# NVIDIA-Merlin/NVTabular

Measured on AMD Instinct MI355X. Metric: rows/sec + GB/s (Criteo Categorify+FillMissing+Normalize fit+transform, HBM-resident), higher is better.
Workload: dtype int32 keys -> int64 labels; fp64 moments/normalize; 1 GPU; synthetic Criteo-day0: 26 int32 categorical (Criteo-1TB cardinalities, Zipf) + 13 int32 continuous, nulls as Arrow bitmaps; Categorify + FillMissing + Normalize, fit + transform; rows_per_gpu=45000000, algorithmic_bytes_per_row=624, tie_break=value (count desc, value asc), artifacts=deferred (no parquet I/O inside the timed region)

## Files before the change

### include/nvt_hip.h

```cpp
#ifndef NVT_HIP_H
#define NVT_HIP_H

#include <stdint.h>

#ifdef __cplusplus
extern "C" {
#endif

#define NVT_OK 0
#define NVT_EINVAL (-1)
#define NVT_EHIP (-2)
#define NVT_ENOMEM (-3)
#define NVT_EUNSUPPORTED (-4)

#define NVT_F32 0
#define NVT_F64 1
#define NVT_I32 2
#define NVT_I64 3
#define NVT_U8 4
#define NVT_I8 5
#define NVT_I16 6

#define NVT_EMPTY_I32 INT32_MIN
#define NVT_EMPTY_I64 INT64_MIN
// ... 278 lines not shown
int nvt_keydir_lookup_image(const void *keys, int dtype, const uint8_t *valid, uint64_t n,
                            const uint32_t *dir, uint64_t dir_slots, const int32_t *keys32, uint64_t nkeys,
                            int64_t key_offset, int64_t null_group, const void *image,
                            uint32_t stride_bytes, int ncols, void *const *outs, const uint8_t *const *folds, const uint32_t *offs,
                            const uint32_t *sizes, const uint64_t *miss_bits, uint64_t *unseen,
                            void *stream);
int nvt_image_build(const nvt_image_part *parts, int nparts, uint64_t records, void *image,
                    uint32_t stride_bytes, void *stream);

int nvt_pq_decode_chunk(const uint8_t *chunk, uint64_t chunk_bytes, int type_size, int max_def_level,
                        uint64_t expect_rows, uint8_t *valid_out, uint64_t valid_bit_offset,
                        uint8_t *values_out, uint64_t values_cap_bytes, uint64_t *rows_out,
                        uint64_t *values_count);
int nvt_pq_decode_chunk_codec(const uint8_t *chunk, uint64_t chunk_bytes, int codec, int type_size,
                              int max_def_level, uint64_t expect_rows, uint8_t *valid_out,
                              uint64_t valid_bit_offset, uint8_t *values_out, uint64_t values_cap_bytes,
                              uint8_t *scratch, uint64_t scratch_bytes, uint64_t *rows_out,
                              uint64_t *values_count);
int nvt_pq_decode_list_chunk(const uint8_t *chunk, uint64_t chunk_bytes, int codec, int type_size,
                             int leaf_level, int max_def_level, uint64_t expect_slots, uint64_t expect_rows,
                             uint8_t *rep_out, uint8_t *def_out, uint64_t slot_offset, uint64_t slot_cap,
                             uint8_t *values_out, uint64_t values_cap_bytes, uint8_t *scratch,
                             uint64_t scratch_bytes, uint64_t *counts);
#define NVT_PQ_RUN_REPEAT 0u
#define NVT_PQ_RUN_PACKED 1u
#define NVT_PQ_RUN_SEQUENCE 2u
#define NVT_PQ_RUN_END 3u
#define NVT_PQ_STR_GROW 1
typedef struct nvt_pq_str_stage {
  int64_t *offsets;
  uint8_t *chars;
  uint32_t *runs;
  uint8_t *packed;
  uint64_t entries_cap, chars_cap, runs_cap, packed_cap;
  uint64_t entries, nchars, nruns, npacked, nvalues;
} nvt_pq_str_stage;
int nvt_pq_decode_str_chunk(const uint8_t *chunk, uint64_t chunk_bytes, int codec, int max_def_level,
                            uint64_t expect_rows, uint8_t *valid_out, uint64_t valid_bit_offset,
                            nvt_pq_str_stage *stage, uint8_t *scratch, uint64_t scratch_bytes, uint64_t *need);
int nvt_pq_expand_runs(const uint32_t *runs, uint64_t nruns, const uint32_t *closing, const uint8_t *packed,
                       uint64_t packed_bytes, uint64_t entries, uint64_t nvalues, int32_t *out, uint32_t *bad,
                       void *stream);
int nvt_expand_valid_ws_bytes(uint64_t n, uint64_t *bytes);
int nvt_expand_valid(const void *packed, int type_size, const uint8_t *bitmap, uint64_t n, void *out,
                     void *ws, void *stream);

typedef struct nvt_moments_col {
  const void *x;
  const uint8_t *valid;
  uint64_t n;
  int32_t dtype, has_fill;
  double fill_val;
  double *out3;
} nvt_moments_col;
int nvt_moments_many(const nvt_moments_col *cols, int ncols, void *partials, void *stream);

typedef struct nvt_fillnorm_col {
  const void *x;
  const uint8_t *valid;
  uint64_t n;
  int32_t dtype, has_fill;
  double fill_val;
  int32_t do_norm, out_dtype;
  double shift, scale;
  void *out;
  uint8_t *filled;
  const double *moments;
} nvt_fillnorm_col;
int nvt_fill_normalize_many(const nvt_fillnorm_col *cols, int ncols, void *stream);

typedef struct nvt_count_col {
  const void *keys;
  const uint8_t *valid;
  const int64_t *weights;
  uint64_t n;
  int32_t key_bytes, path;
  void *ws;
  void *out_keys;
  int64_t *out_counts;
  uint64_t out_capacity;
  uint64_t *state;
  int32_t *hot_image;
  void *range_table;
} nvt_count_col;
int nvt_range_table_bytes(int nb_log2, uint64_t *bytes);
int nvt_dense_count_many(const nvt_count_col *cols, int ncols, void *stream);

typedef struct nvt_vocab_col {
  void *keys;
  int64_t *counts;
  uint64_t n;
  int64_t max_count;
  int32_t key_bytes, unique_keys;
  void *sort_tmp;
  int64_t first_label;
  void *table;
  uint64_t capacity;
  int64_t *sentinel_label;
  void *ready_event;
  const void *src_keys;
  const int64_t *src_counts;
  const uint32_t *cls_hist;
  uint64_t n_big;
  const int32_t *range_aux;
  int32_t range_nb_log2;
  uint64_t flat_slots;
  const int32_t *src_labels;
  void *head_image;
} nvt_vocab_col;
#define NVT_ENCODE_HEAD_BYTES (12288 * 12 + 64)
#define NVT_FLAT_AUX_WORDS (NVT_RANGE_AUX_LO + 16)
#define NVT_FLAT_AUX_MAXDISP (NVT_RANGE_AUX_LO + 8)
#define NVT_FLAT_AUX_NULLGROUP (NVT_RANGE_AUX_LO + 10)
int nvt_vocab_order_tmp_bytes(uint64_t n, uint64_t n_big, uint64_t *bytes);
int nvt_vocab_label_shard(const int32_t *keys, const int64_t *counts, uint64_t n, const uint32_t *class_base_diff,
                          void *tmp, int32_t *label_of, int32_t *big_keys, int64_t *big_counts,
                          int32_t *big_src, void *stream);
int nvt_class_hist(const int64_t *counts, uint64_t n, uint32_t *hist, void *stream);
int nvt_vocab_finalize_many(const nvt_vocab_col *cols, int ncols, void *stream);

typedef struct nvt_encode_col {
  const void *keys;
  const uint8_t *valid;
  uint64_t n;
  const void *table;
  uint64_t capacity;
  const int64_t *sentinel_label;
  int64_t null_label, oov_label;
  uint32_t num_buckets;
  int32_t key_bytes, out_bytes;
  void *out;
  const void *vocab_keys;
  uint64_t n_vocab;
  int64_t first_label;
  void *wait_event;
  const int32_t *range_aux;
  const void *head_image;
} nvt_encode_col;
int nvt_encode_many(const nvt_encode_col *cols, int ncols, void *stream);

int nvt_event_create(void **event);
void nvt_event_destroy(void *event);
int nvt_stream_wait_event(void *stream, void *event);

typedef struct nvt_mailbox nvt_mailbox;
int nvt_mailbox_create(uint64_t bytes, nvt_mailbox **out);
void nvt_mailbox_destroy(nvt_mailbox *mb);
void *nvt_mailbox_data(nvt_mailbox *mb);
uint64_t nvt_mailbox_capacity(nvt_mailbox *mb);
int nvt_mailbox_post(nvt_mailbox *mb, const void *src_device, uint64_t bytes, void *stream,
                     uint64_t *seq_out);
int nvt_mailbox_wait(nvt_mailbox *mb, uint64_t seq, double timeout_s);

int nvt_prof_begin(void);
int nvt_prof_report(char *buf, uint64_t cap, uint64_t *needed);
void nvt_range_push(const char *name);
void nvt_range_pop(void);

int nvt_str_hash(const void *offsets, int offset_bytes, const uint8_t *chars, const uint8_t *valid,
                 uint64_t n, int64_t *out, void *stream);
int nvt_str_take_keys(const int64_t *dict_keys, uint64_t n_dict, const void *indices, int index_bytes,
                      const uint8_t *valid, uint64_t n, int64_t *out, void *stream);
int nvt_str_dedup_ws_bytes(uint64_t n, uint64_t *bytes);
int nvt_str_dedup(const int64_t *keys, const uint8_t *valid, uint64_t n, const void *index, int index_bytes,
                  const void *offsets, int offset_bytes, const uint8_t *chars, uint64_t n_strings, void *ws,
                  uint64_t ws_bytes, int64_t *out_keys, int64_t *out_strs, uint64_t *out_counts,
                  void *stream);
int nvt_str_gather_ws_bytes(uint64_t m, uint64_t *bytes);
int nvt_str_gather(const int64_t *strs, uint64_t m, const void *offsets, int offset_bytes,
                   const uint8_t *chars, uint64_t n_strings, void *ws, uint64_t ws_bytes,
                   int64_t *out_offsets, uint8_t *out_chars, uint64_t out_capacity, void *stream);

#define NVT_COMPACT_MAX_COLS 64
typedef struct nvt_dropna_col {
  const void *x;
  const uint8_t *valid;
  int32_t dtype;
  int32_t reserved;
} nvt_dropna_col;
typedef struct nvt_compact_col {
  const void *src;
  void *dst;
  const uint8_t *src_valid;
  uint8_t *dst_valid;
  const void *plan;
  uint64_t n;
  int32_t width;
  int32_t reserved;
} nvt_compact_col;
int nvt_compact_ws_bytes(uint64_t n, uint64_t *bytes);
int nvt_compact_keep_mask(const uint8_t *mask, uint64_t n, void *ws, uint64_t ws_bytes, void *stream);
// ... 354 lines not shown
```

### nvtabular_amd/_lib.py

```python
from __future__ import annotations

import ctypes as C
import os
import threading

_HERE = os.path.dirname(os.path.abspath(__file__))
LIB_PATH = os.environ.get("NVT_HIP_LIB") or os.path.join(_HERE, "libnvt_hip.so")

NVT_F32, NVT_F64, NVT_I32, NVT_I64, NVT_U8 = 0, 1, 2, 3, 4
NVT_I8, NVT_I16 = 5, 6
NVT_GB_SUMSQ, NVT_GB_MINMAX = 1, 2
NVT_EINVAL, NVT_EHIP, NVT_ENOMEM, NVT_EUNSUPPORTED = -1, -2, -3, -4
ENCODE_HEAD_BYTES = 12288 * 12 + 64
ST_NULLS, ST_SENTINEL, ST_OCCUPIED, ST_OVERFLOW, ST_ROWS = 0, 1, 2, 3, 4
ST_MAXCOUNT = 8
ST_BIG = 9
ST_NEED = 10
STATE_WORDS = 16

_vp, _u64, _i64, _i32, _u32, _dbl = (
    C.c_void_p,
    C.c_uint64,
    C.c_int64,
    C.c_int,
# ... 55 lines not shown
    "nvt_order_rows_ws_bytes": [_u64, C.POINTER(_u64)],
    "nvt_order_rows": [_vp, _vp, _u64, _vp, _u64, _vp, _vp, _vp],
    "nvt_seg_aggregate": [_vp, _u64, _u64, _pp, C.POINTER(C.c_int), _pp, _i32, _vp, _vp, _vp, _vp,
                          _vp, _vp, _vp],
    "nvt_seg_nunique_ws_bytes": [_u64, C.POINTER(_u64)],
    "nvt_seg_nunique": [_vp, _u64, _u64, _pp, C.POINTER(C.c_int), _pp, _i32, _vp, _vp, _vp],
    "nvt_gather_f64": [_vp, _vp, _u64, _dbl, _vp, _i32, _vp],
    "nvt_te_apply": [_vp, _vp, _vp, _vp, _vp, _vp, _u64, _dbl, _dbl, _vp, _i32, _vp],
    "nvt_te_apply_folds": [_vp, _vp, _i32, _vp, _vp, _vp, _vp, _u64, _dbl, _dbl, _vp, _i32, _vp],
    "nvt_sgb_sort_ws_bytes": [_u64, C.POINTER(_u64)],
    "nvt_key_minmax": [_vp, _i32, _u64, _vp, _vp],
    "nvt_sgb_sort": [_vp, _i32, _i64, _vp, _i32, _u64, _vp, C.POINTER(_vp), C.POINTER(C.c_int), _vp],
    "nvt_sgb_regroup_ws_bytes": [_u64, C.POINTER(_u64)],
    "nvt_sgb_regroup": [_vp, _i32, _i32, _i64, _u64, _u64, _vp, _vp, _vp, _vp, _vp, _vp],
    "nvt_sgb_reduce": [_vp, _i32, _i32, _pp, C.POINTER(C.c_int), _pp, _i32, _i32, _u64, _u64,
                       _vp, _vp, _vp, _vp, _vp, _vp, _vp, _vp, _vp, _pp, _pp, _vp],
    "nvt_flat_lookup_gather": [_vp, _i32, _vp, _u64, _vp, _vp, _u64, _i64, _vp, _i32, _pp,
                               C.POINTER(C.c_int), C.POINTER(_dbl), _vp, _vp],
    "nvt_flat_lookup_te": [_vp, _i32, _vp, _u64, _vp, _vp, _u64, _i64, _vp, _i32, _vp, _dbl, _dbl, _vp,
                           _i32, _vp],
    "nvt_flat_lookup_image": [_vp, _i32, _vp, _u64, _vp, _vp, _u64, _i64, _vp, _vp, _vp, _u32, _i32, _pp,
                              _pp, C.POINTER(_u32), C.POINTER(_u32), C.POINTER(_u64), _vp, _vp],
    "nvt_image_pack": [_pp, C.POINTER(C.c_int), C.POINTER(C.c_int), C.POINTER(_u32), _i32, _u64, _vp,
                       _u32, _vp],
    "nvt_jg_image": [_vp, _pp, _pp, _pp, _pp, _i32, C.POINTER(C.c_int), C.POINTER(C.c_int), C.POINTER(C.c_int),
                     C.POINTER(_u32), _i32, _u64, _vp, _u32, _vp],
    "nvt_te_image": [_vp, _vp, _vp, _vp, _i32, _u64, _dbl, _dbl, _i32, _vp, _u32, _u32, _vp],
    "nvt_fold_mt19937_par_ws_bytes": [_u64, _i32, C.POINTER(_u64)],
    "nvt_fold_mt19937_par": [_u32, _i32, _u64, _vp, _vp, _u64, _vp, _vp],
    "nvt_encode_stats": [C.POINTER(_u64), _i32, _vp],
    "nvt_pq_decode_chunk": [_vp, _u64, _i32, _i32, _u64, _vp, _u64, _vp, _u64, C.POINTER(_u64), C.POINTER(_u64)],
    "nvt_pq_decode_chunk_codec": [_vp, _u64, _i32, _i32, _i32, _u64, _vp, _u64, _vp, _u64, _vp, _u64,
                                  C.POINTER(_u64), C.POINTER(_u64)],
    "nvt_pq_decode_list_chunk": [_vp, _u64, _i32, _i32, _i32, _i32, _u64, _u64, _vp, _vp, _u64, _u64, _vp, _u64,
                                 _vp, _u64, C.POINTER(_u64)],
    "nvt_pq_decode_str_chunk": [_vp, _u64, _i32, _i32, _u64, _vp, _u64, _vp, _vp, _u64, C.POINTER(_u64)],
    "nvt_pq_expand_runs": [_vp, _u64, _vp, _vp, _u64, _u64, _u64, _vp, _vp, _vp],
    "nvt_expand_valid_ws_bytes": [_u64, C.POINTER(_u64)],
    "nvt_expand_valid": [_vp, _i32, _vp, _u64, _vp, _vp, _vp],
    "nvt_exchange_ranges": [_vp, _i32, _vp, _vp],
    "nvt_exchange_ranges_sorted": [_vp, _i32, _vp, _vp],
    "nvt_exchange_hist": [_vp, _i32, C.POINTER(_i64), C.POINTER(_u64), _i32, _vp, _vp],
    "nvt_exchange_scatter": [_vp, _i32, C.POINTER(_i64), C.POINTER(_u64), _i32, _vp, _vp, _vp],
    "nvt_exchange_pack_ordered": [_vp, _i32, C.POINTER(_i64), C.POINTER(_u64), _i32, _vp, _vp, _vp, _vp],
    "nvt_exchange_unpack": [_vp, _u64, _vp, _vp, _i32, _vp, _vp, _vp],
    "nvt_count_merge_sorted_ws_bytes": [_u64, C.POINTER(_u64)],
    "nvt_count_merge_sorted": [_vp, _u64, _vp, _i32, _i32, _vp, _vp, _vp, _vp, _vp, _vp],
    "nvt_flat_index_tmp_bytes": [_u64, C.POINTER(_u64)],
    "nvt_flat_index_build": [_vp, _u64, _u64, _vp, _vp, _u64, _vp, _vp],
    "nvt_flat_lookup": [_vp, _i32, _vp, _u64, _vp, _vp, _u64, _i64, _vp, _vp],
    "nvt_widen_i64": [_vp, _i32, _u64, _vp, _vp],
    "nvt_popcount": [_vp, _u64, _vp, _vp],
    "nvt_fold_mt19937": [_u32, _i32, _u64, _vp, _vp],
    "nvt_prefix_distinct": [_vp, _i32, _vp, _vp],
    "nvt_vocab_label_shard": [_vp, _vp, _u64, _vp, _vp, _vp, _vp, _vp, _vp, _vp],
    "nvt_exchange_unpack2": [_vp, _vp, _u64, _vp, _vp, _i32, _vp, _vp, _vp, _vp],
}


class PrefixCol(C.Structure):
    _fields_ = [("keys", _vp), ("valid", _vp), ("n", _u64), ("key_bytes", _i32)]


class XCol(C.Structure):
    _fields_ = [("keys", _vp), ("counts", _vp), ("n", _u64)]


class MomentsCol(C.Structure):
    _fields_ = [("x", _vp), ("valid", _vp), ("n", _u64), ("dtype", C.c_int32),
                ("has_fill", C.c_int32), ("fill_val", _dbl), ("out3", _vp)]


class FillNormCol(C.Structure):
    _fields_ = [("x", _vp), ("valid", _vp), ("n", _u64), ("dtype", C.c_int32),
                ("has_fill", C.c_int32), ("fill_val", _dbl), ("do_norm", C.c_int32),
                ("out_dtype", C.c_int32), ("shift", _dbl), ("scale", _dbl), ("out", _vp),
                ("filled", _vp), ("moments", _vp)]


class CountCol(C.Structure):
    _fields_ = [("keys", _vp), ("valid", _vp), ("weights", _vp), ("n", _u64),
                ("key_bytes", C.c_int32), ("path", C.c_int32), ("ws", _vp), ("out_keys", _vp),
                ("out_counts", _vp), ("out_capacity", _u64), ("state", _vp), ("hot_image", _vp),
                ("range_table", _vp)]


class VocabCol(C.Structure):
    _fields_ = [("keys", _vp), ("counts", _vp), ("n", _u64), ("max_count", _i64),
                ("key_bytes", C.c_int32), ("unique_keys", C.c_int32), ("sort_tmp", _vp),
                ("first_label", _i64), ("table", _vp), ("capacity", _u64),
                ("sentinel_label", _vp), ("ready_event", _vp), ("src_keys", _vp),
                ("src_counts", _vp), ("cls_hist", _vp), ("n_big", _u64), ("range_aux", _vp),
                ("range_nb_log2", C.c_int32), ("flat_slots", C.c_uint64), ("src_labels", _vp),
                ("head_image", _vp)]


class MergeCol(C.Structure):
    _fields_ = [("a_keys", _vp), ("a_counts", _vp), ("na", _u64), ("b_keys", _vp),
                ("b_counts", _vp), ("nb", _u64), ("out_keys", _vp), ("out_counts", _vp),
                ("src_a", _vp), ("src_b", _vp), ("out_n", _vp)]


class PqStrStage(C.Structure):
    _fields_ = [("offsets", _vp), ("chars", _vp), ("runs", _vp), ("packed", _vp),
                ("entries_cap", _u64), ("chars_cap", _u64), ("runs_cap", _u64), ("packed_cap", _u64),
                ("entries", _u64), ("nchars", _u64), ("nruns", _u64), ("npacked", _u64), ("nvalues", _u64)]


PQ_RUN_REPEAT, PQ_RUN_PACKED, PQ_RUN_SEQUENCE, PQ_RUN_END = 0, 1, 2, 3
PQ_STR_GROW = 1


class ImagePart(C.Structure):
    _fields_ = [("kind", C.c_int32), ("nvals", C.c_int32), ("ncols", C.c_int32), ("kfold", C.c_int32),
                ("out_dtype", C.c_int32), ("offset", C.c_uint32), ("groups", _u64), ("count", _vp),
                ("sum", _vp), ("sumsq", _vp), ("mn", _vp), ("mx", _vp), ("kinds", _vp), ("vals", _vp),
                ("dst_dtypes", _vp), ("offs", _vp), ("tot_count", _vp), ("tot_sum", _vp),
                ("fold_count", _vp), ("fold_sum", _vp), ("p_smooth", _dbl), ("y_mean", _dbl),
                ("moments", _vp)]


IMAGE_PART_JG, IMAGE_PART_TE = 0, 1
IMAGE_BUILD_MAX_PARTS, IMAGE_BUILD_MAX_STRIDE = 4, 192


class EncodeCol(C.Structure):
    _fields_ = [("keys", _vp), ("valid", _vp), ("n", _u64), ("table", _vp), ("capacity", _u64),
                ("sentinel_label", _vp), ("null_label", _i64), ("oov_label", _i64),
                ("num_buckets", _u32), ("key_bytes", C.c_int32), ("out_bytes", C.c_int32),
                ("out", _vp), ("vocab_keys", _vp), ("n_vocab", _u64), ("first_label", _i64),
                ("wait_event", _vp), ("range_aux", _vp), ("head_image", _vp)]


SIGNATURES.update({
    "nvt_keydir_build": [_vp, _u64, _u64, _vp, _vp],
    "nvt_keydir_lookup_image": [_vp, _i32, _vp, _u64, _vp, _u64, _vp, _u64, _i64, _i64, _vp, _u32, _i32, _pp,
                                _pp, C.POINTER(_u32), C.POINTER(_u32), C.POINTER(_u64), _vp, _vp],
    "nvt_image_build": [C.POINTER(ImagePart), _i32, _u64, _vp, _u32, _vp],
    "nvt_moments_many": [C.POINTER(MomentsCol), _i32, _vp, _vp],
    "nvt_fill_normalize_many": [C.POINTER(FillNormCol), _i32, _vp],
    "nvt_dense_count_many": [C.POINTER(CountCol), _i32, _vp],
    "nvt_vocab_finalize_many": [C.POINTER(VocabCol), _i32, _vp],
    "nvt_encode_many": [C.POINTER(EncodeCol), _i32, _vp],
    "nvt_merge_sorted_ws_bytes": [C.POINTER(MergeCol), _i32, C.POINTER(_u64)],
    "nvt_merge_sorted_many": [C.POINTER(MergeCol), _i32, _vp, _u64, _vp],
    "nvt_merge_payload": [_vp, _vp, _u64, _i32, _i32, _i32, _vp, _vp, _vp, _vp],
    "nvt_event_create": [_pp],
    "nvt_event_destroy": [_vp],
    "nvt_stream_wait_event": [_vp, _vp],
    "nvt_mailbox_create": [_u64, _pp],
    "nvt_mailbox_destroy": [_vp],
    "nvt_mailbox_data": [_vp],
    "nvt_mailbox_capacity": [_vp],
    "nvt_mailbox_post": [_vp, _vp, _u64, _vp, C.POINTER(_u64)],
    "nvt_mailbox_wait": [_vp, _u64, _dbl],
    "nvt_prof_begin": [],
    "nvt_prof_report": [C.c_char_p, _u64, C.POINTER(_u64)],
    "nvt_range_push": [C.c_char_p],
    "nvt_range_pop": [],
    "nvt_str_hash": [_vp, _i32, _vp, _vp, _u64, _vp, _vp],
    "nvt_str_take_keys": [_vp, _u64, _vp, _i32, _vp, _u64, _vp, _vp],
    "nvt_str_dedup_ws_bytes": [_u64, C.POINTER(_u64)],
    "nvt_str_dedup": [_vp, _vp, _u64, _vp, _i32, _vp, _i32, _vp, _u64, _vp, _u64, _vp, _vp, _vp, _vp],
    "nvt_str_gather_ws_bytes": [_u64, C.POINTER(_u64)],
    "nvt_str_gather": [_vp, _u64, _vp, _i32, _vp, _u64, _vp, _u64, _vp, _vp, _u64, _vp],
})


class DropnaCol(C.Structure):
    _fields_ = [("x", _vp), ("valid", _vp), ("dtype", C.c_int32), ("reserved", C.c_int32)]


class CompactCol(C.Structure):
    _fields_ = [("src", _vp), ("dst", _vp), ("src_valid", _vp), ("dst_valid", _vp), ("plan", _vp),
                ("n", _u64), ("width", C.c_int32), ("reserved", C.c_int32)]


# ... 282 lines not shown
```

### nvtabular_amd/csrc/nvt_dense_count.hip

```cpp
#include <algorithm>
#include <vector>

#include "nvt_common.hpp"
#include "nvt_internal.hpp"
#include "nvt_prof.hpp"
#include "nvt_range.hpp"

namespace nvt {

struct CountPath {
  int kind;
  bool hot, pieces;
  int nb_log2;
};

static const char *count_path(int path, int key_bytes, bool weighted, CountPath *p) {
  if (key_bytes != 4 && key_bytes != 8) return "key_bytes must be 4 or 8";
  *p = {path & 0xFF, false, false, 0};
  if (p->kind == NVT_PATH_SORT) {
    if (key_bytes != 4 || weighted) return "the sort path takes int32 keys without weights";
    return nullptr;
  }
  if (p->kind == NVT_PATH_RANGE) {
    if (key_bytes != 4 || weighted) return "the range path takes int32 keys without weights";
    p->nb_log2 = (path >> 8) & 0xFF;
    p->pieces = (path & NVT_PATH_PIECES) != 0;
    if (p->nb_log2 < 6 || p->nb_log2 > 10) return "range path: 64 .. 1024 buckets";
    return nullptr;
  }
  p->hot = (path & NVT_PATH_HOT) != 0;
  p->kind = path & ~NVT_PATH_HOT;
  const bool parted = p->kind >= 1 && p->kind <= 3;
  if (!(p->kind == 0 || p->kind == 6 || p->kind == 7 || parted))
    return "path must be 0 / 6 / 7 (LDS tables: one key class / tiny / two key classes) or "
           "1 / 2 / 3 (partitioned)";
  if (p->hot && !(parted && key_bytes == 4 && !weighted))
    return "the hot filter takes int32 keys without weights on paths 1 / 2 / 3";
  return nullptr;
}

static const char *count_col_check(const CountPath &p, const nvt_count_col &c) {
  if (!c.state || !c.ws) return "null state/workspace";
  if (p.kind == NVT_PATH_RANGE && !c.hot_image)
    return "the range path needs the column's aux block (nvt_dense_count_many, hot_image)";
  if (p.kind == NVT_PATH_SORT && !c.hot_image)
    return "the sort path needs the column's histogram block";
  if (reinterpret_cast<uintptr_t>(c.keys) & 15) return "keys must be 16-byte aligned";
  if (c.n && !(c.keys && c.out_keys && c.out_counts)) return "null keys/out";
  if (p.kind != NVT_PATH_SORT && c.n >= (1ull << 32))
    return "at most 2^32-1 rows per call (32-bit LDS counters)";
  return nullptr;
}

static uint64_t dense_ws_layout(const CountPath &p, int key_bytes, uint64_t n, bool weighted) {
  if (p.kind == NVT_PATH_SORT) return sort_count_ws_bytes(n);
  if (p.kind == NVT_PATH_RANGE) return range_count_ws_bytes(n, p.nb_log2);
  if (p.kind >= 1 && p.kind <= 3) return part_count_ws_bytes(p.kind, p.hot, key_bytes, weighted, n);
  return lds_count_ws_bytes(p.kind, key_bytes, weighted);
}

static const char *prof_name(const CountPath &p) {
  static const char *const kPlain[8] = {"dense_count_p0", "dense_count_p1", "dense_count_p2",
                                        "dense_count_p3", nullptr,          nullptr,
                                        "dense_count_p6", "dense_count_p7"};
  static const char *const kHot[4] = {nullptr, "dense_count_h1", "dense_count_h2", "dense_count_h3"};
  return p.hot ? kHot[p.kind] : kPlain[p.kind];
}

template <typename K>
static int dense_count(const CountPath &p, const nvt_count_col &c, hipStream_t s) {
  if (p.kind >= 1 && p.kind <= 3) return part_count<K>(c, p.kind, p.hot, s);
  return lds_count<K>(c, p.kind, s);
}

static int count_column(const CountPath &p, const nvt_count_col &c, hipStream_t s, bool clear_state) {
  if (p.kind == NVT_PATH_SORT || p.kind == NVT_PATH_RANGE) {
    if (clear_state) NVT_CHECK_HIP(hipMemsetAsync(c.state, 0, NVT_STATE_WORDS * 8, s));
    if (c.n == 0) return NVT_OK;
    if (p.kind == NVT_PATH_SORT)
      return sort_count_i32((const int32_t *)c.keys, c.valid, c.n, c.ws, (unsigned *)c.hot_image,
                            (int32_t *)c.out_keys, c.out_counts, c.out_capacity, c.state, s);
    return range_count_i32((const int32_t *)c.keys, c.valid, c.n, p.nb_log2, c.ws, c.hot_image,
                           (int32_t *)c.out_keys, c.out_counts, c.out_capacity, c.range_table,
                           c.state, s, p.pieces);
  }
  NVT_PROF(prof_name(p), c.n * c.key_bytes, s);
  if (clear_state) NVT_CHECK_HIP(hipMemsetAsync(c.state, 0, NVT_STATE_WORDS * 8, s));
  if (c.n == 0) return NVT_OK;
  return c.key_bytes == 4 ? dense_count<int32_t>(p, c, s) : dense_count<int64_t>(p, c, s);
}

static int count_single(const void *keys, const uint8_t *valid, const int64_t *weights, uint64_t n,
                        int key_bytes, int path, void *ws, void *out_keys, int64_t *out_counts,
                        uint64_t out_capacity, uint64_t *state, void *stream) {
  nvt_count_col c = {};
  c.keys = keys, c.valid = valid, c.weights = weights, c.n = n;
  c.key_bytes = key_bytes, c.path = path, c.ws = ws, c.state = state;
  c.out_keys = out_keys, c.out_counts = out_counts, c.out_capacity = out_capacity;
  CountPath p;
  const char *why = count_path(path, key_bytes, weights != nullptr, &p);
  if (!why) why = count_col_check(p, c);
  if (why) {
    set_error("dense_count: %s", why);
    return NVT_EINVAL;
  }
  return count_column(p, c, (hipStream_t)stream, true);
}

}

using namespace nvt;

extern "C" {

int nvt_range_table_bytes(int nb_log2, uint64_t *bytes) {
  NVT_CHECK_ARG(bytes && nb_log2 >= 6 && nb_log2 <= 10, "64 .. 1024 buckets");
  *bytes = (((uint64_t)1 << nb_log2) * kRpRegion + kRpGuard) * 8;
  return NVT_OK;
}
int nvt_dense_count_ws_bytes(int key_bytes, uint64_t n, int path, int weighted, uint64_t *bytes) {
  NVT_CHECK_ARG(bytes, "null bytes");
  CountPath p;
  if (const char *why = count_path(path, key_bytes, weighted != 0, &p)) {
    set_error("%s: %s", __func__, why);
    return NVT_EINVAL;
  }
  *bytes = dense_ws_layout(p, key_bytes, n, weighted != 0) + 64;
  return NVT_OK;
}
int nvt_dense_count_many(const nvt_count_col *cols, int ncols, void *stream) {
  NVT_CHECK_ARG(ncols == 0 || cols, "null descriptors");
  hipStream_t main_s = (hipStream_t)stream;
  std::vector<void *> wss;
  for (int i = 0; i < ncols; ++i)
    if (std::find(wss.begin(), wss.end(), cols[i].ws) == wss.end()) wss.push_back(cols[i].ws);
  if (wss.size() > (size_t)kSideStreams) {
    set_error("nvt_dense_count_many: at most %d distinct workspaces per call", kSideStreams);
    return NVT_EINVAL;
  }
  std::vector<CountPath> paths(std::max(ncols, 0));
  for (int i = 0; i < ncols; ++i) {
    const char *why = count_path(cols[i].path, cols[i].key_bytes, cols[i].weights != nullptr, &paths[i]);
    if (!why) why = count_col_check(paths[i], cols[i]);
    if (why) {
      set_error("nvt_dense_count_many: %s (column %d)", why, i);
      return NVT_EINVAL;
    }
  }
  bool contiguous = ncols > 1;
  for (int i = 0; i < ncols && contiguous; ++i)
    contiguous = cols[i].state == cols[0].state + (uint64_t)i * NVT_STATE_WORDS;
  if (contiguous)
    NVT_CHECK_HIP(hipMemsetAsync(cols[0].state, 0, (uint64_t)ncols * NVT_STATE_WORDS * 8, main_s));
  SidePool *pool = nullptr;
  const bool fork = wss.size() > 1;
  if (fork) {
    int rc = side_pool(1, &pool);
    if (rc) return rc;
    NVT_CHECK_HIP(hipEventRecord(pool->fork, main_s));
    for (size_t k = 0; k < wss.size(); ++k) NVT_CHECK_HIP(hipStreamWaitEvent(pool->s[k], pool->fork, 0));
  }
  auto sampled_here = [&](int i) {
    return (paths[i].hot || paths[i].kind == NVT_PATH_RANGE) && cols[i].hot_image && cols[i].n != 0;
  };
  bool sampled = false;
  {
    HotSampleBatch hb;
// ... 66 lines not shown
```

### nvtabular_amd/csrc/nvt_finalize.hip

```cpp
#include <algorithm>
#include <cstdlib>
#include <mutex>
#include <vector>

#include "nvt_common.hpp"
#include "nvt_internal.hpp"
#include "nvt_prof.hpp"

namespace nvt {
namespace {
constexpr int kSide = kSideStreams;
constexpr uint64_t kOrderBatchMaxEntries = 1ull << 23;
}
}

using namespace nvt;

static int finalize_impl(const nvt_vocab_col *cols, int ncols, hipStream_t main_s, SidePool *&pool,
                         bool &forked);

extern "C" int nvt_vocab_finalize_many(const nvt_vocab_col *cols, int ncols, void *stream) {
  NVT_CHECK_ARG(ncols == 0 || cols, "null descriptors");
  SidePool *pool = nullptr;
  bool forked = false;
  const int rc = finalize_impl(cols, ncols, (hipStream_t)stream, pool, forked);
  if (rc != NVT_OK && forked && pool != nullptr) {
    for (int i = 0; i < kSide; ++i) {
      (void)hipEventRecord(pool->join[i], pool->s[i]);
      (void)hipStreamWaitEvent((hipStream_t)stream, pool->join[i], 0);
    }
  }
  return rc;
}

static int finalize_impl(const nvt_vocab_col *cols, int ncols, hipStream_t main_s, SidePool *&pool,
                         bool &forked) {
  std::vector<int> small, big;
  for (int i = 0; i < ncols; ++i) {
    const nvt_vocab_col &c = cols[i];
    NVT_CHECK_ARG(c.key_bytes == 4 || c.key_bytes == 8, "key_bytes must be 4 or 8");
    NVT_CHECK_ARG(c.n <= 1 || (c.keys && c.counts), "null keys/counts");
    NVT_CHECK_ARG(c.table == nullptr || c.sentinel_label, "table without sentinel_label");
    NVT_CHECK_ARG(c.src_keys == nullptr || (c.key_bytes == 4 && c.src_counts && (c.cls_hist || c.src_labels)),
                  "key-sorted source: int32 keys with src_counts and cls_hist (or src_labels)");
    if (c.src_keys == nullptr && vocab_sort_small_eligible(c.key_bytes, c.n, c.max_count))
      small.push_back(i);
    else
      big.push_back(i);
  }
  std::sort(big.begin(), big.end(), [&](int a, int b) { return cols[a].n > cols[b].n; });
  const bool fork = big.size() + (small.empty() ? 0 : 1) > 1 && !getenv("NVT_FINALIZE_SERIAL");
  if (fork) {
    int rc = side_pool(0, &pool);
    if (rc) return rc;
    forked = true;
    NVT_CHECK_HIP(hipEventRecord(pool->fork, main_s));
    for (int i = 0; i < kSide; ++i) NVT_CHECK_HIP(hipStreamWaitEvent(pool->s[i], pool->fork, 0));
  }
  bool need_join = false;
  auto build_heads = [&](const std::vector<int> &which, hipStream_t s) -> int {
    std::vector<const int32_t *> k;
    std::vector<uint64_t> nn;
    std::vector<int64_t> fl;
    std::vector<void *> im;
    for (int i : which) {
      const nvt_vocab_col &c = cols[i];
      if (!(c.head_image && c.key_bytes == 4 && c.unique_keys)) continue;
      k.push_back((const int32_t *)c.keys);
      nn.push_back(c.n);
      fl.push_back(c.first_label);
      im.push_back(c.head_image);
    }
    if (k.empty()) return NVT_OK;
    return encode_head_build_many(k.data(), nn.data(), fl.data(), im.data(), (int)k.size(), s);
  };
  auto finish = [&](const nvt_vocab_col &c, hipStream_t s, bool head = true) -> int {
    if (c.table != nullptr && c.src_keys == nullptr) {
      int rc = encode_build_any(c.key_bytes, c.keys, c.n, c.first_label, c.table, c.capacity,
                                c.sentinel_label, c.unique_keys, s);
      if (rc) return rc;
    }
    if (head && c.head_image && c.key_bytes == 4 && c.unique_keys) {
      int rc = encode_head_build((const int32_t *)c.keys, c.n, c.first_label, c.head_image, s);
      if (rc) return rc;
    }
    if (c.ready_event) {
      NVT_CHECK_HIP(hipEventRecord((hipEvent_t)c.ready_event, s));
    } else if (s != main_s)
      need_join = true;
    return NVT_OK;
  };
  if (!small.empty()) {
    std::vector<SmallSortDesc> d(small.size());
    for (size_t j = 0; j < small.size(); ++j) {
      const nvt_vocab_col &c = cols[small[j]];
      d[j].keys = (int32_t *)c.keys;
      d[j].counts = c.counts;
      d[j].n = (unsigned)c.n;
    }
    int rc = vocab_sort_small_batch(d.data(), (int)d.size(), main_s);
    if (rc) return rc;
    for (int i : small) {
      rc = finish(cols[i], main_s);
      if (rc) return rc;
    }
  }
  std::vector<OrderTail> tails;
  std::vector<int> tail_cols;
  std::vector<char> batched(ncols > 0 ? ncols : 0, 0);
  {
    std::vector<OrderSortedJob> jobs;
    std::vector<int> job_cols;
    for (int i : big) {
      const nvt_vocab_col &c = cols[i];
      if (c.src_keys == nullptr || c.table == nullptr || c.range_aux == nullptr || c.n == 0) continue;
      if (c.src_labels != nullptr) continue;
      if (c.n > kOrderBatchMaxEntries) continue;
      NVT_CHECK_ARG(c.sort_tmp, "null sort_tmp");
      jobs.push_back({(const int32_t *)c.src_keys, c.src_counts, c.n, c.cls_hist, c.n_big, c.max_count,
                      (int32_t *)c.keys, c.counts, c.sort_tmp, c.first_label, c.table, c.capacity,
                      c.sentinel_label, c.range_aux, c.range_nb_log2, c.flat_slots});
      job_cols.push_back(i);
      batched[i] = 1;
    }
    if (!jobs.empty()) {
      hipStream_t s = fork ? pool->s[0] : main_s;
      int rc = vocab_order_sorted_batch(jobs.data(), (int)jobs.size(), s);
      if (rc) return rc;
      rc = build_heads(job_cols, s);
      if (rc) return rc;
      for (int i : job_cols) {
        rc = finish(cols[i], s, false);
        if (rc) return rc;
      }
    }
  }
  for (size_t j = 0; j < big.size(); ++j) {
    const nvt_vocab_col &c = cols[big[j]];
    if (batched[big[j]]) continue;
    hipStream_t s = fork ? pool->s[j % kSide] : main_s;
    if (c.src_keys != nullptr && c.src_labels != nullptr) {
      NVT_CHECK_ARG(c.sort_tmp, "null sort_tmp");
      int rc = vocab_from_labels((const int32_t *)c.src_keys, c.src_counts, c.src_labels, c.n,
                                 (int32_t *)c.keys, c.counts, c.sort_tmp, c.first_label, c.table,
                                 c.capacity, c.sentinel_label, c.range_aux, c.flat_slots, s);
      if (rc) return rc;
      if (c.head_image && c.key_bytes == 4 && c.unique_keys) {
        rc = encode_head_build((const int32_t *)c.keys, c.n, c.first_label, c.head_image, s);
        if (rc) return rc;
      }
      if (c.ready_event) {
        NVT_CHECK_HIP(hipEventRecord((hipEvent_t)c.ready_event, s));
      } else if (s != main_s)
        need_join = true;
      continue;
    }
    if (c.src_keys != nullptr) {
      NVT_CHECK_ARG(c.sort_tmp, "null sort_tmp");
      bool deferred = false;
      int rc = vocab_order_from_sorted((const int32_t *)c.src_keys, c.src_counts, c.n, c.cls_hist,
                                       c.n_big, c.max_count, (int32_t *)c.keys, c.counts,
                                       c.sort_tmp, c.first_label, c.table, c.capacity,
                                       c.sentinel_label, c.range_aux, c.range_nb_log2, s,
                                       &deferred, c.flat_slots);
      if (rc) return rc;
      if (deferred) {
        tails.push_back({(int32_t *)c.keys, c.counts, c.n_big, c.first_label, c.table, c.capacity,
                         c.sentinel_label, c.range_aux});
        tail_cols.push_back(big[j]);
        continue;
      }
    } else if (c.n > 1) {
      NVT_CHECK_ARG(c.sort_tmp, "null sort_tmp");
      int rc = vocab_sort_any(c.key_bytes, c.keys, c.counts, c.n, c.max_count, c.sort_tmp, s);
      if (rc) return rc;
    }
    int rc = finish(c, s);
    if (rc) return rc;
  }
  if (!tails.empty()) {
    hipStream_t ts = main_s;
    bool all_events = true;
    for (int i : tail_cols) all_events = all_events && cols[i].ready_event != nullptr;
    if (fork) {
      ts = pool->s[0];
      for (int i = 1; i < kSide; ++i) {
        NVT_CHECK_HIP(hipEventRecord(pool->join[i], pool->s[i]));
        NVT_CHECK_HIP(hipStreamWaitEvent(ts, pool->join[i], 0));
      }
      if (!all_events) need_join = true;
    }
    int rc = vocab_order_tail_batch(tails.data(), (int)tails.size(), ts);
    if (rc) return rc;
    rc = build_heads(tail_cols, ts);
    if (rc) return rc;
    for (int i : tail_cols)
      if (cols[i].ready_event) NVT_CHECK_HIP(hipEventRecord((hipEvent_t)cols[i].ready_event, ts));
  }
  if (fork && need_join) {
    for (int i = 0; i < kSide; ++i) {
      NVT_CHECK_HIP(hipEventRecord(pool->join[i], pool->s[i]));
      NVT_CHECK_HIP(hipStreamWaitEvent(main_s, pool->join[i], 0));
    }
  }
  return NVT_OK;
}

extern "C" int nvt_event_create(void **event) {
  NVT_CHECK_ARG(event, "null out pointer");
  hipEvent_t e = nullptr;
  NVT_CHECK_HIP(hipEventCreateWithFlags(&e, getenv("NVT_EVENT_TIMING") ? hipEventDefault
                                                                        : hipEventDisableTiming));
  *event = (void *)e;
  return NVT_OK;
}
extern "C" void nvt_event_destroy(void *event) {
  if (event) (void)hipEventDestroy((hipEvent_t)event);
}
extern "C" int nvt_stream_wait_event(void *stream, void *event) {
  NVT_CHECK_ARG(event, "null event");
  NVT_CHECK_HIP(hipStreamWaitEvent((hipStream_t)stream, (hipEvent_t)event, 0));
  return NVT_OK;
}
```

### nvtabular_amd/csrc/nvt_internal.hpp

```cpp
#pragma once
#include <hip/hip_runtime.h>
#include <stdint.h>

#include "../../include/nvt_hip.h"

namespace nvt {

constexpr int kSideStreams = 3;
struct SidePool {
  int dev = -1, which = 0;
  hipStream_t s[kSideStreams];
  hipEvent_t fork, join[kSideStreams], aux;
};
int side_pool(int which, SidePool **out);

int vocab_sort_any(int key_bytes, void *keys, int64_t *counts, uint64_t n, int64_t max_count,
                   void *tmp, hipStream_t s);
struct SmallSortDesc {
  int32_t *keys;
  int64_t *counts;
  unsigned n;
};
bool vocab_sort_small_eligible(int key_bytes, uint64_t n, int64_t max_count);
int vocab_sort_small_batch(const SmallSortDesc *cols, int ncols, hipStream_t s);

uint64_t sort_words_tmp_bytes(uint64_t n);
int sort_words_bits(uint64_t *data, uint64_t n, int bit_lo, int bit_hi, void *tmp, uint64_t **result,
                    hipStream_t s);
int sort_packed_keys(const void *keys, int key_dtype, int64_t key_bias, const uint8_t *fold, int rb,
                     uint64_t n, void *tmp, uint64_t **result, hipStream_t stream);

struct HotSampleCol {
  const int32_t *keys;
  const uint8_t *valid;
  uint64_t n;
  int32_t *image;
  int nb_log2;
  int pieces;
};
constexpr int kHotBatch = 32;
struct HotSampleBatch {
  HotSampleCol c[kHotBatch];
};
int hot_sample_launch(const HotSampleBatch &batch, int ncols, hipStream_t s);

uint64_t lds_count_ws_bytes(int kind, int key_bytes, bool weighted);
template <typename K>
int lds_count(const nvt_count_col &c, int kind, hipStream_t s);

uint64_t part_count_ws_bytes(int kind, bool hot, int key_bytes, bool weighted, uint64_t n);
template <typename K>
int part_count(const nvt_count_col &c, int kind, bool hot, hipStream_t s);

uint64_t range_count_ws_bytes(uint64_t n, int nb_log2);
int range_count_i32(const int32_t *keys, const uint8_t *valid, uint64_t n, int nb_log2, void *ws,
                    int32_t *aux, int32_t *out_keys, int64_t *out_cnt, uint64_t out_cap,
                    void *range_table, uint64_t *state, hipStream_t s, bool pieces);

uint64_t sort_count_ws_bytes(uint64_t n);
int sort_count_i32(const int32_t *keys, const uint8_t *valid, uint64_t n, void *ws, unsigned *hist,
                   int32_t *out_keys, int64_t *out_cnt, uint64_t out_cap, uint64_t *state,
                   hipStream_t s);

uint64_t vocab_order_tmp_bytes(uint64_t n, uint64_t n_big);
int vocab_order_from_sorted(const int32_t *src_keys, const int64_t *src_cnts, uint64_t n,
                            const unsigned *cls_hist, uint64_t n_big, int64_t max_count,
                            int32_t *out_keys, int64_t *out_cnts, void *tmp, int64_t first_label,
                            void *table, uint64_t capacity, int64_t *sentinel_label,
                            const int32_t *range_aux, int range_nb_log2, hipStream_t s,
                            bool *tail_deferred, uint64_t flat_slots = 0);
struct OrderSortedJob {
  const int32_t *src_keys;
  const int64_t *src_cnts;
  uint64_t n;
  const unsigned *cls_hist;
  uint64_t n_big;
  int64_t max_count;
  int32_t *out_keys;
  int64_t *out_cnts;
  void *tmp;
  int64_t first_label;
  void *table;
  uint64_t capacity;
  int64_t *sentinel_label;
  const int32_t *range_aux;
  int range_nb_log2;
  uint64_t flat_slots;
};
int vocab_order_sorted_batch(const OrderSortedJob *jobs, int njobs, hipStream_t s);
int encode_head_build(const int32_t *vocab_keys, uint64_t n, int64_t first_label, void *image,
                      hipStream_t s);
int encode_head_build_many(const int32_t *const *vocab_keys, const uint64_t *n, const int64_t *first_label,
                           void *const *images, int count, hipStream_t s);
int vocab_from_labels(const int32_t *src_keys, const int64_t *src_cnts, const int32_t *labels, uint64_t n,
                      int32_t *out_keys, int64_t *out_cnts, void *tmp, int64_t first_label, void *table,
                      uint64_t capacity, int64_t *sentinel_label, const int32_t *range_aux,
                      uint64_t flat_slots, hipStream_t s);
struct OrderTail {
  int32_t *keys;
  int64_t *counts;
  uint64_t n_big;
  int64_t first_label;
  void *table;
  uint64_t capacity;
  int64_t *sentinel_label;
  const int32_t *range_aux;
};
int vocab_order_tail_batch(const OrderTail *t, int nt, hipStream_t s);

int encode_clear_any(int key_bytes, void *table, uint64_t capacity, int64_t *sentinel_label,
                     hipStream_t s);
int encode_insert_any(int key_bytes, const void *vocab, uint64_t n, int64_t first_label,
                      void *table, uint64_t capacity, int64_t *sentinel_label, hipStream_t s);
int encode_build_any(int key_bytes, const void *vocab, uint64_t n, int64_t first_label, void *table,
                     uint64_t capacity, int64_t *sentinel_label, int unique_keys, hipStream_t s);

}
```

### nvtabular_amd/csrc/nvt_range_count.hip

```cpp
#include <cstdio>
#include <cstdlib>
#include <type_traits>

#include "nvt_common.hpp"
#include "nvt_internal.hpp"
#include "nvt_prof.hpp"
#include "nvt_range.hpp"

namespace nvt {

namespace {

constexpr int32_t kEmpty = INT32_MIN;
constexpr int kRpBS = 1024;
constexpr int kRpG = NVT_RANGE_WGS;
constexpr int kRpBinWords = 20480;
constexpr int kRpLine = 16;
constexpr int kRpMaxNbLog2 = 10;
constexpr int kHotSlotsR = NVT_HOT_IMAGE_WORDS;
constexpr int kHotBucketsR = kHotSlotsR / 2;
constexpr int kRpProbe = 512;
#ifndef NVT_RP_MAX_EPOCH
#define NVT_RP_MAX_EPOCH 8
#endif
// ... 221 lines not shown
      if ((pend >> q) & 1) {
        const unsigned bkt = rp_fine<PW>(map, kv[q]) >> 14;
        const unsigned pos = atomicAdd(&fill[bkt], 1u);
        if (pos < CAP) {
          bins[bkt * CAP + pos] = kv[q];
        } else {
          const unsigned at = flushed[bkt] + pos;
          if (at < region_cap)
            regions[((uint64_t)bkt * kRpG + g) * region_cap + at] = kv[q];
          else
            atomicOr(&s_ovf, 1u);
        }
      }
    }
    if (++since >= R) {
      __syncthreads();
      flush_bins(false, epoch & 1u);
      if (threadIdx.x == 0) s_epoch[(epoch + 1u) & 1u] = 0;
      __syncthreads();
      const unsigned fl = s_epoch[epoch & 1u];
#ifndef NVT_RP_GROW_DIV
#define NVT_RP_GROW_DIV 16u
#endif
#ifndef NVT_RP_SHRINK_DIV
#define NVT_RP_SHRINK_DIV 4u
#endif
      if ((fl >> 8) > NB / NVT_RP_SHRINK_DIV) R = R > 1u ? R / 2u : 1u;
      else if ((fl >> 8) <= NB / NVT_RP_GROW_DIV) R = R < kRpMaxEpoch ? R * 2u : R;
      ++epoch;
      since = 0;
    }
  }
  __syncthreads();
  flush_bins(true, epoch & 1u);
  __syncthreads();
  for (unsigned b = threadIdx.x; b < NB; b += kRpBS) fills[(uint64_t)b * kRpG + g] = flushed[b];
  for (int i = threadIdx.x; i < kHotBucketsR; i += kRpBS) {
    const int4 hbk = hot[i];
    reinterpret_cast<uint2 *>(hot_cnt + (uint64_t)g * kHotSlotsR)[i] = make_uint2((unsigned)hbk.z, (unsigned)hbk.w);
  }
#pragma unroll
  for (int off = 32; off > 0; off >>= 1) {
    nulls += __shfl_down(nulls, off, 64);
    notvalid += __shfl_down(notvalid, off, 64);
  }
  if (lane == 0) {
    if (nulls) atomicAdd(&s_nulls, nulls);
    const unsigned long long sent = empties - notvalid;
    if (sent) atomicAdd(&s_sent, sent);
  }
  __syncthreads();
  if (threadIdx.x == 0) {
    if (s_nulls) atomicAdd((unsigned long long *)&state[NVT_ST_NULLS], s_nulls);
    if (s_sent) atomicAdd((unsigned long long *)&state[NVT_ST_SENTINEL], s_sent);
    if (s_ovf) atomicOr((unsigned long long *)&state[NVT_ST_OVERFLOW], 1ull | NVT_OVF_REGION);
    if (g == 0) atomicAdd((unsigned long long *)&state[NVT_ST_ROWS], (unsigned long long)n);
  }
}

constexpr int kTotGroups = 16;
__global__ __launch_bounds__(64 * kTotGroups) void hot_totals_kernel(
    const unsigned *__restrict__ hot_cnt, int nblocks, unsigned *__restrict__ hot_tot) {
  __shared__ unsigned part[kTotGroups][64];
  const unsigned l = threadIdx.x & 63, g = threadIdx.x >> 6;
  const unsigned slot = blockIdx.x * 64 + l;
  unsigned t = 0;
#pragma unroll 16
  for (int b = (int)g; b < nblocks; b += kTotGroups) t += hot_cnt[(uint64_t)b * kHotSlotsR + slot];
  part[g][l] = t;
  __syncthreads();
  if (g != 0) return;
  unsigned tot = 0;
#pragma unroll
  for (int q = 0; q < kTotGroups; ++q) tot += part[q][l];
  hot_tot[slot] = tot;
}

template <bool PW>
__global__ __launch_bounds__(kRpBS) void rp_count_kernel(
    const int32_t *__restrict__ regions, const uint32_t *__restrict__ fills, uint32_t region_cap,
    const int32_t *__restrict__ aux, const unsigned *__restrict__ hot_tot, int nb_log2,
    unsigned long long *status, unsigned *ticket, int32_t *__restrict__ out_keys,
    int64_t *__restrict__ out_cnt, uint64_t out_cap, unsigned *cls_hist,
    unsigned long long *__restrict__ range_table, uint64_t *state) {
  constexpr int NSL = kRpSlots + kRpTail;
  constexpr int NW = kRpBS / kWave;
  __shared__ int32_t lkeys[NSL];
  __shared__ unsigned lcnt[NSL];
  __shared__ unsigned run_len[kRpG];
  __shared__ unsigned hist[256];
  __shared__ unsigned wtot[NW];
  __shared__ unsigned lovf, s_b, s_bad, s_mx;
  __shared__ unsigned long long s_base;
  if (threadIdx.x == 0) {
    s_b = atomicAdd(ticket, 1u);
    lovf = 0;
    s_mx = 0;
  }
  for (int i = threadIdx.x; i < NSL; i += kRpBS) {
    lkeys[i] = kEmpty;
    lcnt[i] = 0;
  }
  if (threadIdx.x < 256) hist[threadIdx.x] = 0;
  __syncthreads();
  const unsigned b = s_b, NB = 1u << nb_log2;
  const unsigned lane = lane_id(), w = threadIdx.x / kWave;
  RangeMap map = load_map(aux);
  __shared__ uint32_t s_pieces[kRpPwWords];
  stage_pieces(map, s_pieces, threadIdx.x, kRpBS);
  const bool skip = (state[NVT_ST_OVERFLOW] & 1ull) != 0;
  if (threadIdx.x < kRpG) {
    const unsigned len = fills[(uint64_t)b * kRpG + threadIdx.x];
    run_len[threadIdx.x] = (skip || len > region_cap) ? 0u : len;
  }
  __syncthreads();
  bool failed = skip;
  auto insert_from = [&](int32_t key, unsigned wgt, uint32_t s) {
#pragma unroll 4
    for (int p = 0; p < kRpProbe; ++p, ++s) {
      if (s >= (uint32_t)NSL) break;
      int32_t cur = lkeys[s];
      if (cur == kEmpty) {
        cur = atomicCAS(&lkeys[s], kEmpty, key);
        if (cur == kEmpty) cur = key;
      }
      if (cur == key) {
        atomicAdd(&lcnt[s], wgt);
        return;
      }
    }
    failed = true;
  };
  const unsigned hot_h0 = (unsigned)aux[NVT_RANGE_AUX_HOTSTART + b], hot_h1 = (unsigned)aux[NVT_RANGE_AUX_HOTSTART + b + 1];
  int32_t hot_key0 = kEmpty;
  unsigned hot_tot0 = 0;
  if (hot_h0 + threadIdx.x < hot_h1) {
    const unsigned slot = reinterpret_cast<const unsigned short *>(aux + NVT_RANGE_AUX_HOTORDER)[hot_h0 + threadIdx.x];
    hot_key0 = aux[slot];
    hot_tot0 = hot_tot[slot];
  }
  {
    __shared__ unsigned s_pre[kRpG + 2];
    __shared__ unsigned s_wsum[kRpG / kWave];
    static_assert(kRpG % kWave == 0 && kRpG <= kRpBS, "one thread per run");
    {
      unsigned len = 0, inc = 0;
      if (threadIdx.x < kRpG) {
        len = run_len[threadIdx.x];
        inc = len;
#pragma unroll
        for (int off = 1; off < 64; off <<= 1) {
          const unsigned o = __shfl_up(inc, off, 64);
          if (lane >= (unsigned)off) inc += o;
        }
        if (lane == 63) s_wsum[w] = inc;
      }
      __syncthreads();
      if (threadIdx.x < kRpG) {
        unsigned wb = 0;
        for (unsigned q = 0; q < w; ++q) wb += s_wsum[q];
        s_pre[threadIdx.x] = wb + inc - len;
        if (threadIdx.x == kRpG - 1) s_pre[kRpG] = wb + inc;
      }
    }
    __syncthreads();
    const unsigned *pre = s_pre;
    const unsigned all_keys = pre[kRpG];
// ... 104 lines not shown
      const int32_t key = aux[slot];
      const unsigned tot = hot_tot[slot];
      if (key != kEmpty && tot > 0 && !failed) insert_from(key, tot, rp_fine<PW>(map, key) & (kRpSlots - 1));
    }
  }
  if (failed) atomicOr(&lovf, 1u);
  __syncthreads();
  if (threadIdx.x == 0)
    s_bad = (lovf != 0 ||
             (__hip_atomic_load(&state[NVT_ST_OVERFLOW], __ATOMIC_RELAXED,
                                __HIP_MEMORY_SCOPE_AGENT) & 1ull))
                ? 1u : 0u;
  __syncthreads();
  const bool bad = s_bad != 0;
  const unsigned long long sent_rows = b == 0 ? state[NVT_ST_SENTINEL] : 0ull;
  const unsigned extra = sent_rows > 0 ? 1u : 0u;
  constexpr int ITER = (NSL + kRpBS - 1) / kRpBS;
  unsigned mine = 0;
  for (int it = 0; it < ITER; ++it) {
    const int i = it * kRpBS + (int)threadIdx.x;
    const bool occ = i < NSL && lkeys[i] != kEmpty;
    mine += (unsigned)__popcll(__ballot(occ));
  }
  if (lane == 0) wtot[w] = mine;
  __syncthreads();
  unsigned E = extra;
  for (int q = 0; q < NW; ++q) E += wtot[q];
  const bool full = E > (unsigned)(kRpSlots / 4 * 3);
  if (bad || full) E = 0;
  if (w == 0) {
    unsigned long long excl = 0;
    if (lane == 0)
      __hip_atomic_store(&status[b], (b == 0 ? kStPrefix : kStAgg) | (unsigned long long)E,
                         __ATOMIC_RELAXED, __HIP_MEMORY_SCOPE_AGENT);
    if (b > 0) {
      int top = (int)b - 1;
      while (true) {
        const int idx = top - (int)lane;
        unsigned long long v = kStPrefix;
        if (idx >= 0) {
          do {
            v = __hip_atomic_load(&status[idx], __ATOMIC_RELAXED, __HIP_MEMORY_SCOPE_AGENT);
#ifndef NVT_RP_SLEEP
#define NVT_RP_SLEEP 1
#endif
            if ((v >> 62) == 0) __builtin_amdgcn_s_sleep(NVT_RP_SLEEP);
          } while ((v >> 62) == 0);
        }
        const unsigned long long isp = __ballot((v >> 62) == 2);
        const int first = isp ? (int)__ffsll((long long)isp) - 1 : 64;
        unsigned long long add = ((int)lane <= first) ? (v & kStMask) : 0ull;
#pragma unroll
        for (int off = 32; off > 0; off >>= 1) add += __shfl_down(add, off, 64);
        excl += __shfl(add, 0, 64);
        if (isp) break;
        top -= 64;
      }
      if (lane == 0)
        __hip_atomic_store(&status[b], kStPrefix | (excl + E), __ATOMIC_RELAXED,
                           __HIP_MEMORY_SCOPE_AGENT);
    }
    if (lane == 0) s_base = excl;
  }
  __syncthreads();
  const unsigned long long base = s_base;
  if (b == NB - 1 && threadIdx.x == 0) {
    if (base + E > out_cap) {
      atomicOr((unsigned long long *)&state[NVT_ST_OVERFLOW], 2ull);
      state[NVT_ST_NEED] = base + E;
    } else {
      state[NVT_ST_OCCUPIED] = base + E;
    }
  }
  if (bad || full) {
    if (threadIdx.x == 0 && (lovf != 0 || full))
      atomicOr((unsigned long long *)&state[NVT_ST_OVERFLOW],
               1ull | (lovf != 0 ? NVT_OVF_PROBE : 0ull) | (full ? NVT_OVF_FULL : 0ull));
    return;
  }
  if (base + E > out_cap) return;
  if (extra && threadIdx.x == 0) {
    out_keys[base] = kEmpty;
    out_cnt[base] = (int64_t)sent_rows;
    const unsigned cls = sent_rows < 255 ? (unsigned)sent_rows : 255u;
    atomicAdd(&hist[cls], 1u);
    unsigned long long *gm = reinterpret_cast<unsigned long long *>(&state[NVT_ST_MAXCOUNT]);
    atomicMax(gm, sent_rows);
  }
  __shared__ unsigned occ_pre[ITER * NW];
  __shared__ unsigned occ_wsum[8];
  for (int it = 0; it < ITER; ++it) {
    const int i = it * kRpBS + (int)threadIdx.x;
    const bool occ = i < NSL && lkeys[i] != kEmpty;
    const unsigned c = (unsigned)__popcll(__ballot(occ));
    if (lane == 0) occ_pre[it * NW + w] = c;
  }
  __syncthreads();
  {
    constexpr int NG = ITER * NW;
    constexpr int SW = (NG + kWave - 1) / kWave;
    unsigned v = 0, inc = 0;
    if (w < (unsigned)SW) {
      v = threadIdx.x < (unsigned)NG ? occ_pre[threadIdx.x] : 0u;
      inc = v;
#pragma unroll
      for (int off = 1; off < 64; off <<= 1) {
        const unsigned o = __shfl_up(inc, off, 64);
        if (lane >= (unsigned)off) inc += o;
      }
      if (lane == 63) occ_wsum[w] = inc;
    }
    __syncthreads();
    if (w < (unsigned)SW && threadIdx.x < (unsigned)NG) {
      unsigned wb = 0;
      for (unsigned q = 0; q < w; ++q) wb += occ_wsum[q];
      occ_pre[threadIdx.x] = extra + wb + inc - v;
    }
    __syncthreads();
  }
  unsigned mx = 0;
  for (int it = 0; it < ITER; ++it) {
    const int i = it * kRpBS + (int)threadIdx.x;
    const int32_t k = i < NSL ? lkeys[i] : kEmpty;
    const bool occ = k != kEmpty;
    unsigned long long dump = kEncEmptySlot;
    const unsigned long long bal = __ballot(occ);
    const unsigned front = occ_pre[it * NW + w];
    if (occ) {
      const unsigned p_i = front + (unsigned)__popcll(bal & ((1ull << lane) - 1ull));
      unsigned rank = 0;
      int s = i;
      while (true) {
        int32_t o[4];
#pragma unroll
        for (int q = 0; q < 4; ++q) o[q] = s - 1 - q >= 0 ? lkeys[s - 1 - q] : kEmpty;
        int run = 0;
        bool open = true;
#pragma unroll
        for (int q = 0; q < 4; ++q) {
          open = open && o[q] != kEmpty;
          run += open ? 1 : 0;
          rank += (open && o[q] < k) ? 1u : 0u;
        }
        s -= run;
        if (run < 4) break;
      }
      int e = i + 1;
      while (true) {
        int32_t o[4];
#pragma unroll
        for (int q = 0; q < 4; ++q) o[q] = e + q < NSL ? lkeys[e + q] : kEmpty;
        int run = 0;
        bool open = true;
#pragma unroll
        for (int q = 0; q < 4; ++q) {
          open = open && o[q] != kEmpty;
          run += open ? 1 : 0;
          rank += (open && o[q] < k) ? 1u : 0u;
        }
        e += run;
        if (run < 4) break;
      }
      const uint64_t pos = base + p_i - (unsigned)(i - s) + rank;
      const unsigned c = lcnt[i];
      out_keys[pos] = k;
      out_cnt[pos] = (int64_t)c;
      atomicAdd(&hist[c < 255u ? c : 255u], 1u);
      mx = c > mx ? c : mx;
      dump = ((unsigned long long)(uint32_t)pos << 32) | (uint32_t)k;
    }
    if (range_table != nullptr && i < NSL) range_table[(uint64_t)b * NSL + i] = dump;
  }
#pragma unroll
  for (int off = 32; off > 0; off >>= 1) {
    const unsigned o = __shfl_down(mx, off, 64);
    mx = o > mx ? o : mx;
  }
  if (lane == 0 && mx > 0) atomicMax(&s_mx, mx);
  if (range_table != nullptr && b == NB - 1 && threadIdx.x < kRpGuard)
    range_table[(uint64_t)NB * NSL + threadIdx.x] = kEncEmptySlot;
  __syncthreads();
  if (threadIdx.x == 0 && s_mx > 0)
    atomicMax(reinterpret_cast<unsigned long long *>(&state[NVT_ST_MAXCOUNT]), (unsigned long long)s_mx);
  if (threadIdx.x < 256) {
    const unsigned h = hist[threadIdx.x];
    if (h) atomicAdd(&cls_hist[threadIdx.x], h);
    if (threadIdx.x == 255 && h)
      atomicAdd((unsigned long long *)&state[NVT_ST_BIG], (unsigned long long)h);
  }
}

inline uint64_t al16(uint64_t x) { return (x + 15) & ~15ull; }

}

uint32_t range_region_cap(uint64_t n, int nb_log2) {
  const uint64_t rows_per_wg = (n + kRpG - 1) / kRpG;
  const uint64_t c = 2 * (rows_per_wg >> nb_log2) + 64;
  return (uint32_t)((c + kRpLine - 1) / kRpLine * kRpLine);
}

struct RangeWs {
  int32_t *regions;
  uint32_t *fills;
  unsigned *hot_cnt, *hot_tot;
  unsigned long long *status;
  unsigned *ticket;
};

uint64_t range_ws_layout(uint64_t n, int nb_log2, char *base, RangeWs *ws) {
  uint64_t off = 0;
  auto take = [&](uint64_t bytes) {
    char *p = base ? base + off : nullptr;
    off += al16(bytes);
    return p;
  };
  RangeWs w;
  const uint64_t NB = 1ull << nb_log2;
  w.regions = (int32_t *)take(NB * kRpG * range_region_cap(n, nb_log2) * 4);
  w.fills = (uint32_t *)take(NB * kRpG * 4);
  w.hot_cnt = (unsigned *)take((uint64_t)kRpG * kHotSlotsR * 4);
  w.hot_tot = (unsigned *)take((uint64_t)kHotSlotsR * 4);
  w.status = (unsigned long long *)take(NB * 8 + 64);
  w.ticket = (unsigned *)(w.status ? (char *)w.status + NB * 8 : nullptr);
  if (ws) *ws = w;
  return off;
}

uint64_t range_count_ws_bytes(uint64_t n, int nb_log2) {
  return range_ws_layout(n, nb_log2, nullptr, nullptr);
}

int range_count_i32(const int32_t *keys, const uint8_t *valid, uint64_t n, int nb_log2, void *wsp,
                    int32_t *aux, int32_t *out_keys, int64_t *out_cnt, uint64_t out_cap,
                    void *range_table, uint64_t *state, hipStream_t s, bool pieces) {
  NVT_CHECK_ARG(nb_log2 >= 6 && nb_log2 <= kRpMaxNbLog2, "range path: 64 .. 1024 buckets");
  NVT_CHECK_ARG(aux != nullptr, "range path: the column needs its aux block (hot_image)");
  NVT_PROF("dense_count_r9", n * 4, s);
  RangeWs w;
  range_ws_layout(n, nb_log2, (char *)wsp, &w);
  const unsigned NB = 1u << nb_log2;
  const uint32_t cap = range_region_cap(n, nb_log2);
  unsigned *hist = (unsigned *)(aux + NVT_RANGE_AUX_HIST);
#define NVT_RP_PART(NBL)                                                                            \
  do {                                                                                              \
    if (pieces)                                                                                     \
      rp_partition_kernel<NVT_RANGE_U, NBL, true><<<kRpG, kRpBS, 0, s>>>(                           \
          keys, valid, n, aux, nb_log2, cap, w.regions, w.fills, w.hot_cnt, state, w.status, hist); \
    else                                                                                            \
      rp_partition_kernel<NVT_RANGE_U, NBL, false><<<kRpG, kRpBS, 0, s>>>(                          \
          keys, valid, n, aux, nb_log2, cap, w.regions, w.fills, w.hot_cnt, state, w.status, hist); \
  } while (0)
  if (nb_log2 == 8) NVT_RP_PART(8);
  else if (nb_log2 == 9) NVT_RP_PART(9);
  else if (nb_log2 == 10) NVT_RP_PART(10);
  else NVT_RP_PART(0);
#undef NVT_RP_PART
  NVT_CHECK_LAUNCH();
  hot_totals_kernel<<<kHotSlotsR / 64, 64 * kTotGroups, 0, s>>>(w.hot_cnt, kRpG, w.hot_tot);
  NVT_CHECK_LAUNCH();
  if (pieces)
    rp_count_kernel<true><<<NB, kRpBS, 0, s>>>(w.regions, w.fills, cap, aux, w.hot_tot, nb_log2, w.status,
                                               w.ticket, out_keys, out_cnt, out_cap,
                                               (unsigned *)(aux + NVT_RANGE_AUX_HIST),
                                               (unsigned long long *)range_table, state);
  else
    rp_count_kernel<false><<<NB, kRpBS, 0, s>>>(w.regions, w.fills, cap, aux, w.hot_tot, nb_log2, w.status,
                                                w.ticket, out_keys, out_cnt, out_cap,
                                                (unsigned *)(aux + NVT_RANGE_AUX_HIST),
                                                (unsigned long long *)range_table, state);
  NVT_CHECK_LAUNCH();
  return NVT_OK;
}

}
```

### nvtabular_amd/csrc/nvt_sort.hip

```cpp
#include <type_traits>

#include <cstdlib>

#include "nvt_common.hpp"
#include "nvt_internal.hpp"
#include "nvt_prof.hpp"
#include "nvt_scan.hpp"
#include "nvt_sort_tile.hpp"

namespace nvt {

template <typename K>
__device__ __forceinline__ unsigned sort_digit(K key, int64_t cnt, int pass) {
  constexpr int KB = (int)sizeof(K);
  if (pass < KB) {
    using U = typename std::make_unsigned<K>::type;
    U u = (U)key ^ ((U)1 << (8 * KB - 1));
    return (unsigned)((u >> (8 * pass)) & 0xFF);
  }
  uint64_t inv = ~(uint64_t)cnt;
  return (unsigned)((inv >> (8 * (pass - KB))) & 0xFF);
}

constexpr int kSmallMax = 8192;
// ... 587 lines not shown
__global__ __launch_bounds__(kS2BS) void os_hist_words_kernel(const uint64_t *__restrict__ w,
                                                              uint64_t n, int bit_lo, int npass,
                                                              unsigned *__restrict__ block_hist) {
  os_hist_words_body([=](uint64_t i) -> uint64_t { return w[i]; }, n, bit_lo, npass, block_hist);
}
template <typename K>
__global__ __launch_bounds__(kS2BS) void os_hist_pack_kernel(PackedKeyWord<K> src, uint64_t n, int bit_lo,
                                                             int npass, unsigned *__restrict__ block_hist) {
  os_hist_words_body(src, n, bit_lo, npass, block_hist);
}

uint64_t sort_words_tmp_bytes(uint64_t n) { return os_tmp_bytes(n); }

static int sort_words_impl(uint64_t *data, const void *keys, int key_dtype, int64_t key_bias,
                           const uint8_t *fold, int rb, uint64_t n, int bit_lo, int bit_hi, void *tmp,
                           uint64_t **result, hipStream_t stream) {
  NVT_CHECK_ARG(n < (1ull << 30), "at most 2^30-1 words");
  const int npass = (bit_hi - bit_lo + 7) / 8;
  NVT_CHECK_ARG(npass >= 1 && npass <= kOsMaxPass, "bit range too wide");
  const uint64_t ntiles = (n + kS2Tile - 1) / kS2Tile;
  char *p = reinterpret_cast<char *>(tmp);
  uint64_t *bufs[2];
  bufs[0] = reinterpret_cast<uint64_t *>(p);
  p += n * 8;
  bufs[1] = reinterpret_cast<uint64_t *>(p);
  p += n * 8;
  unsigned *block_hist = reinterpret_cast<unsigned *>(p);
  p += (uint64_t)kOsHistBlocks * kOsMaxPass * 256 * 4;
  unsigned *base = reinterpret_cast<unsigned *>(p);
  p += kOsMaxPass * 256 * 4;
  unsigned *status = reinterpret_cast<unsigned *>(p);
  const uint64_t status_words = (uint64_t)npass * ntiles * 256;
  unsigned *tickets = status + status_words;
  NVT_CHECK_HIP(hipMemsetAsync(status, 0, (status_words + kOsMaxPass) * 4, stream));
  const unsigned hb = (unsigned)(ntiles < (uint64_t)kOsHistBlocks ? ntiles : kOsHistBlocks);
  const PackedKeyWord<int32_t> s32{reinterpret_cast<const int32_t *>(keys), fold, key_bias, rb};
  const PackedKeyWord<int64_t> s64{reinterpret_cast<const int64_t *>(keys), fold, key_bias, rb};
  if (!keys)
    os_hist_words_kernel<<<hb, kS2BS, 0, stream>>>(data, n, bit_lo, npass, block_hist);
  else if (key_dtype == NVT_I32)
    os_hist_pack_kernel<int32_t><<<hb, kS2BS, 0, stream>>>(s32, n, bit_lo, npass, block_hist);
  else
    os_hist_pack_kernel<int64_t><<<hb, kS2BS, 0, stream>>>(s64, n, bit_lo, npass, block_hist);
  NVT_CHECK_LAUNCH();
  os_base_kernel<<<npass, 256, 0, stream>>>(block_hist, (int)hb, base);
  NVT_CHECK_LAUNCH();
  const uint64_t *src = data;
  int flip = 0;
  for (int pass = 0; pass < npass; ++pass) {
    uint64_t *dst = bufs[flip];
    unsigned *st = status + (uint64_t)pass * ntiles * 256;
    if (pass == 0 && keys && key_dtype == NVT_I32)
      os_scatter_pack_kernel<int32_t><<<(unsigned)ntiles, kS2BS, 0, stream>>>(
          s32, n, bit_lo, base, st, tickets, dst);
    else if (pass == 0 && keys)
      os_scatter_pack_kernel<int64_t><<<(unsigned)ntiles, kS2BS, 0, stream>>>(
          s64, n, bit_lo, base, st, tickets, dst);
    else
      os_scatter_kernel<false, false><<<(unsigned)ntiles, kS2BS, 0, stream>>>(
          src, nullptr, nullptr, n, bit_lo + 8 * pass, base + pass * 256, st, tickets + pass, dst,
          nullptr, nullptr);
    NVT_CHECK_LAUNCH();
    src = dst;
    flip ^= 1;
  }
  *result = const_cast<uint64_t *>(src);
  return NVT_OK;
}

int sort_words_bits(uint64_t *data, uint64_t n, int bit_lo, int bit_hi, void *tmp, uint64_t **result,
                    hipStream_t stream) {
  *result = data;
  if (n <= 1 || bit_hi <= bit_lo) return NVT_OK;
  return sort_words_impl(data, nullptr, 0, 0, nullptr, 0, n, bit_lo, bit_hi, tmp, result, stream);
}

int sort_packed_keys(const void *keys, int key_dtype, int64_t key_bias, const uint8_t *fold, int rb,
                     uint64_t n, void *tmp, uint64_t **result, hipStream_t stream) {
  NVT_CHECK_ARG(keys && n >= 1 && rb >= 24 && rb <= 32, "keys / rows / row bits");
  return sort_words_impl(nullptr, keys, key_dtype, key_bias, fold, rb, n, rb, 64, tmp, result, stream);
}

constexpr int kSmallPackedMax = 16384;
struct SmallCol {
  int32_t *keys;
  int64_t *counts;
  unsigned n;
};
constexpr int kSmallBatch = 64;
struct SmallBatch {
  SmallCol c[kSmallBatch];
};
__global__ __launch_bounds__(kSmallBS) void sort_small_packed_many_kernel(SmallBatch b) {
  __shared__ uint64_t sv[kSmallPackedMax];
  const SmallCol col = b.c[blockIdx.x];
  const unsigned n = col.n;
  unsigned m = 1;
  while (m < n) m <<= 1;
  for (unsigned i = threadIdx.x; i < m; i += kSmallBS)
    sv[i] = i < n ? comp_make(col.keys[i], col.counts[i]) : ~0ull;
  __syncthreads();
  for (unsigned size = 2; size <= m; size <<= 1) {
    for (unsigned stride = size >> 1; stride > 0; stride >>= 1) {
      for (unsigned t = threadIdx.x; t < m / 2; t += kSmallBS) {
        const unsigned lo = 2 * t - (t & (stride - 1));
        const unsigned hi = lo + stride;
        const bool up = (lo & size) == 0;
        const uint64_t a = sv[lo], c = sv[hi];
        if (up ? (c < a) : (a < c)) {
          sv[lo] = c;
          sv[hi] = a;
        }
      }
      __syncthreads();
    }
  }
  for (unsigned i = threadIdx.x; i < n; i += kSmallBS) {
    const uint64_t v = sv[i];
    col.keys[i] = comp_key(v);
    col.counts[i] = comp_cnt(v);
  }
}

inline uint64_t sort2_tmp_bytes(uint64_t n) {
  const uint64_t ntiles = (n + kS2Tile - 1) / kS2Tile, hist_len = 256 * ntiles;
  return 2 * n * 8 + pad16(hist_len * 4) + scan_chunks(hist_len) * 8 + 64;
}

inline int vocab_sort_packed(int32_t *keys, int64_t *counts, uint64_t n, int64_t max_count,
                             void *tmp, hipStream_t stream) {
  const uint64_t ntiles = (n + kS2Tile - 1) / kS2Tile, hist_len = 256 * ntiles;
  char *p = reinterpret_cast<char *>(tmp);
  uint64_t *bufs[2];
  bufs[0] = reinterpret_cast<uint64_t *>(p);
  p += n * 8;
  bufs[1] = reinterpret_cast<uint64_t *>(p);
  p += n * 8;
  unsigned *tile_hist = reinterpret_cast<unsigned *>(p);
  p += pad16(hist_len * 4);
  unsigned long long *chunk_tot = reinterpret_cast<unsigned long long *>(p);
  int count_bytes = 0;
  for (uint64_t m = (uint64_t)max_count; m; m >>= 8) ++count_bytes;
  const int npass = 4 + count_bytes;
  const uint64_t *src = nullptr;
  int flip = 0;
  for (int pass = 0; pass < npass; ++pass) {
    const int shift = 8 * pass;
    const bool first = pass == 0, last = pass == npass - 1;
    if (first)
      sort2_hist_kernel<true><<<(unsigned)ntiles, kS2BS, 0, stream>>>(nullptr, keys, counts, n,
                                                                       shift, tile_hist, ntiles);
    else
      sort2_hist_kernel<false><<<(unsigned)ntiles, kS2BS, 0, stream>>>(src, nullptr, nullptr, n,
                                                                        shift, tile_hist, ntiles);
    NVT_CHECK_LAUNCH();
    const unsigned long long *cbase = nullptr;
    {
      int rc = exclusive_scan_u32_deferred(tile_hist, hist_len, chunk_tot, &cbase, stream);
      if (rc) return rc;
    }
    uint64_t *dst = bufs[flip];
    if (first)
      sort2_scatter_kernel<true, false><<<(unsigned)ntiles, kS2BS, 0, stream>>>(
          nullptr, keys, counts, n, shift, tile_hist, cbase, ntiles, dst, nullptr, nullptr);
    else if (last)
      sort2_scatter_kernel<false, true><<<(unsigned)ntiles, kS2BS, 0, stream>>>(
          src, nullptr, nullptr, n, shift, tile_hist, cbase, ntiles, nullptr, keys, counts);
    else
      sort2_scatter_kernel<false, false><<<(unsigned)ntiles, kS2BS, 0, stream>>>(
          src, nullptr, nullptr, n, shift, tile_hist, cbase, ntiles, dst, nullptr, nullptr);
    NVT_CHECK_LAUNCH();
    src = dst;
    flip ^= 1;
  }
  return NVT_OK;
}

template <typename K>
int vocab_sort(K *keys, int64_t *counts, uint64_t n, int64_t max_count, void *tmp,
               hipStream_t stream) {
  constexpr int NP = (int)sizeof(K) + 8;
  if (n <= 1) return NVT_OK;
  NVT_CHECK_ARG(n < (1ull << 32), "at most 2^32-1 vocabulary entries");
  if (n <= kSmallMax) {
    sort_small_kernel<K><<<1, kSmallBS, 0, stream>>>(keys, counts, (unsigned)n);
    NVT_CHECK_LAUNCH();
    return NVT_OK;
  }
  if constexpr (sizeof(K) == 4) {
    if (max_count > 0 && max_count < (1ll << 32) && n < (1ull << 30))
      return vocab_sort_onesweep(keys, counts, n, max_count, tmp, stream);
    if (max_count > 0 && max_count < (1ll << 32) && n < (1ull << 31))
      return vocab_sort_packed(keys, counts, n, max_count, tmp, stream);
  }
  const uint64_t ntiles = (n + kTileSort - 1) / kTileSort;
  char *p = reinterpret_cast<char *>(tmp);
  int64_t *counts2 = reinterpret_cast<int64_t *>(p);
  p += n * sizeof(int64_t);
  K *keys2 = reinterpret_cast<K *>(p);
  p += pad16(n * sizeof(K));
  unsigned *tile_hist = reinterpret_cast<unsigned *>(p);
  const uint64_t hist_len = 256 * ntiles;
  p += pad16(hist_len * sizeof(unsigned));
  const uint64_t nchunks = (hist_len + kScanChunk - 1) / kScanChunk;
  unsigned long long *chunk_tot = reinterpret_cast<unsigned long long *>(p);
  p += nchunks * sizeof(unsigned long long);
  unsigned long long *pass_hist = reinterpret_cast<unsigned long long *>(p);

  bool run_pass[NP];
  if (max_count > 0) {
    constexpr int KB = (int)sizeof(K);
    int count_bytes = 0;
    for (uint64_t m = (uint64_t)max_count; m; m >>= 8) ++count_bytes;
    for (int p = 0; p < NP; ++p) run_pass[p] = p < KB || (p - KB) < count_bytes;
  } else {
    NVT_CHECK_HIP(hipMemsetAsync(pass_hist, 0, NP * 256 * sizeof(unsigned long long), stream));
    sort_pass_hist_kernel<K><<<stream_grid(n, kBlock * 8, 4), kBlock, 0, stream>>>(keys, counts, n,
                                                                                     pass_hist);
    NVT_CHECK_LAUNCH();
    unsigned long long host_hist[NP * 256];
    NVT_CHECK_HIP(hipMemcpyAsync(host_hist, pass_hist, sizeof(host_hist), hipMemcpyDeviceToHost,
                                 stream));
    NVT_CHECK_HIP(hipStreamSynchronize(stream));
    for (int p = 0; p < NP; ++p) {
      run_pass[p] = true;
      for (int d = 0; d < 256; ++d)
        if (host_hist[p * 256 + d] == n) run_pass[p] = false;
    }
  }

  K *src_k = keys, *dst_k = keys2;
  int64_t *src_c = counts, *dst_c = counts2;
  for (int pass = 0; pass < NP; ++pass) {
    if (!run_pass[pass]) continue;
    sort_tile_hist_kernel<K><<<(unsigned)ntiles, kBlock, 0, stream>>>(src_k, src_c, n, pass,
                                                                      tile_hist, ntiles);
    NVT_CHECK_LAUNCH();
    {
      int rc = exclusive_scan_u32(tile_hist, hist_len, chunk_tot, stream);
      if (rc) return rc;
    }
    sort_scatter_kernel<K><<<(unsigned)ntiles, kBlock, 0, stream>>>(src_k, src_c, n, pass,
                                                                    tile_hist, ntiles, dst_k, dst_c);
    NVT_CHECK_LAUNCH();
    K *tk = src_k;
    src_k = dst_k;
    dst_k = tk;
    int64_t *tc = src_c;
    src_c = dst_c;
    dst_c = tc;
  }
  if (src_k != keys) {
    NVT_CHECK_HIP(hipMemcpyAsync(keys, src_k, n * sizeof(K), hipMemcpyDeviceToDevice, stream));
    NVT_CHECK_HIP(
        hipMemcpyAsync(counts, src_c, n * sizeof(int64_t), hipMemcpyDeviceToDevice, stream));
  }
  return NVT_OK;
}

int vocab_sort_any(int key_bytes, void *keys, int64_t *counts, uint64_t n, int64_t max_count,
                   void *tmp, hipStream_t s) {
  NVT_PROF("vocab_sort", 0, s);
  if (key_bytes == 4) return vocab_sort<int32_t>((int32_t *)keys, counts, n, max_count, tmp, s);
  return vocab_sort<int64_t>((int64_t *)keys, counts, n, max_count, tmp, s);
}

bool vocab_sort_small_eligible(int key_bytes, uint64_t n, int64_t max_count) {
  return key_bytes == 4 && n >= 2 && n <= (uint64_t)kSmallPackedMax && max_count > 0 &&
         max_count < (1ll << 32);
}

int vocab_sort_small_batch(const SmallSortDesc *cols, int ncols, hipStream_t s) {
  for (int c0 = 0; c0 < ncols; c0 += kSmallBatch) {
    const int nc = ncols - c0 < kSmallBatch ? ncols - c0 : kSmallBatch;
    SmallBatch b;
    memset(&b, 0, sizeof(b));
    for (int i = 0; i < nc; ++i) {
      b.c[i].keys = cols[c0 + i].keys;
      b.c[i].counts = cols[c0 + i].counts;
      b.c[i].n = cols[c0 + i].n;
    }
    NVT_PROF("vocab_sort_small", 0, s);
    sort_small_packed_many_kernel<<<nc, kSmallBS, 0, s>>>(b);
    NVT_CHECK_LAUNCH();
  }
  return NVT_OK;
}

}

using namespace nvt;

extern "C" {

int nvt_vocab_sort_tmp_bytes(int key_bytes, uint64_t n, uint64_t *bytes) {
  NVT_CHECK_ARG(bytes && (key_bytes == 4 || key_bytes == 8), "key_bytes must be 4 or 8");
  const uint64_t ntiles = (n + kTileSort - 1) / kTileSort;
  const uint64_t hist_len = 256 * ntiles;
  const uint64_t nchunks = (hist_len + kScanChunk - 1) / kScanChunk;
  *bytes = n * 8 + pad16(n * key_bytes) + pad16(hist_len * 4) + nchunks * 8 +
           (uint64_t)(key_bytes + 8) * 256 * 8 + 64;
  if (key_bytes == 4 && sort2_tmp_bytes(n) > *bytes) *bytes = sort2_tmp_bytes(n);
  if (key_bytes == 4 && os_tmp_bytes(n) > *bytes) *bytes = os_tmp_bytes(n);
  return NVT_OK;
}
int nvt_vocab_sort_i32(int32_t *keys, int64_t *counts, uint64_t n, int64_t max_count, void *tmp,
                       void *stream) {
  NVT_CHECK_ARG(n <= 1 || (keys && counts && tmp), "null pointer");
  return vocab_sort_any(4, keys, counts, n, max_count, tmp, (hipStream_t)stream);
}
int nvt_vocab_sort_i64(int64_t *keys, int64_t *counts, uint64_t n, int64_t max_count, void *tmp,
                       void *stream) {
  NVT_CHECK_ARG(n <= 1 || (keys && counts && tmp), "null pointer");
  return vocab_sort_any(8, keys, counts, n, max_count, tmp, (hipStream_t)stream);
}

}
```

### nvtabular_amd/csrc/nvt_vocab_order.hip

```cpp
#include <vector>

#include "nvt_common.hpp"
#include "nvt_internal.hpp"
#include "nvt_prof.hpp"
#include "nvt_range.hpp"
#include "nvt_sort_tile.hpp"

namespace nvt {

__device__ __forceinline__ unsigned cls_digit(uint64_t comp) {
  const uint32_t cnt = ~(uint32_t)(comp >> 32);
  return 255u - (cnt < 255u ? cnt : 255u);
}

__device__ __forceinline__ void cls_scatter_body(
    const int32_t *__restrict__ keys, const int64_t *__restrict__ cnts, uint64_t n,
    const unsigned *__restrict__ cls_hist, unsigned *status, unsigned *ticket, int32_t *out_keys,
    int64_t *out_cnts, unsigned long long *table, uint64_t mask, int64_t first_label,
    int64_t *sentinel_label, int32_t *label_of, int32_t *big_src = nullptr) {
  constexpr int NW = kS2BS / kWave;
  __shared__ unsigned wcnt[NW][256];
  __shared__ unsigned goff[256];
  __shared__ unsigned wtot[NW], btot[NW];
  __shared__ unsigned s_tile;
  __shared__ uint64_t stage[kS2Tile];
  const unsigned w = threadIdx.x / kWave, l = lane_id();
  if (threadIdx.x == 0) s_tile = atomicAdd(ticket, 1u);
#pragma unroll
  for (int q = 0; q < NW; ++q) wcnt[q][threadIdx.x] = 0;
  unsigned cbase;
  {
    const unsigned v = cls_hist[255 - threadIdx.x];
    unsigned inc = v;
#pragma unroll
    for (int off = 1; off < 64; off <<= 1) {
      unsigned o = __shfl_up(inc, off, 64);
      if (l >= (unsigned)off) inc += o;
    }
    if (l == 63) btot[w] = inc;
    __syncthreads();
    unsigned wb = 0;
    for (unsigned q = 0; q < w; ++q) wb += btot[q];
    cbase = wb + inc - v;
  }
  const unsigned tile = s_tile;
  uint64_t c[kS2Rows];
  unsigned short local[kS2Rows];
#pragma unroll
  for (int r = 0; r < kS2Rows; ++r) {
    const uint64_t i = s2_elem(tile, w, r, l);
    c[r] = ~0ull;
    if (i < n) {
      const int64_t cn = cnts[i];
      c[r] = comp_make(keys[i], cn > 0xFFFFFFFFll ? 0xFFFFFFFFll : cn);
    }
  }
  const uint64_t tile_base = (uint64_t)tile * kS2Tile;
#pragma unroll
  for (int r = 0; r < kS2Rows; ++r) {
    const bool act = s2_elem(tile, w, r, l) < n;
    const unsigned d = cls_digit(c[r]);
    const unsigned long long peers = match_digit(d, act);
    const unsigned rank = __popcll(peers & ((1ull << l) - 1ull));
    const unsigned before = act ? wcnt[w][d] : 0;
    __builtin_amdgcn_wave_barrier();
    if (act && rank == 0) wcnt[w][d] = before + (unsigned)__popcll(peers);
    __builtin_amdgcn_wave_barrier();
    local[r] = (unsigned short)(before + rank);
  }
  __syncthreads();
  {
    const unsigned d = threadIdx.x;
    unsigned t[NW], tot = 0;
#pragma unroll
    for (int q = 0; q < NW; ++q) {
      t[q] = wcnt[q][d];
      tot += t[q];
    }
    unsigned *my = status + (uint64_t)tile * 256 + d;
    __hip_atomic_store(my, (tile == 0 ? kOsPrefix : kOsAgg) | tot, __ATOMIC_RELAXED,
                       __HIP_MEMORY_SCOPE_AGENT);
    unsigned inc = tot;
#pragma unroll
    for (int off = 1; off < 64; off <<= 1) {
      unsigned o = __shfl_up(inc, off, 64);
      if (l >= (unsigned)off) inc += o;
    }
    if (l == 63) wtot[w] = inc;
    __syncthreads();
    unsigned wbase = 0;
    for (unsigned q = 0; q < w; ++q) wbase += wtot[q];
    const unsigned dstart = wbase + inc - tot;
    unsigned run = dstart;
#pragma unroll
    for (int q = 0; q < NW; ++q) {
      wcnt[q][d] = run;
      run += t[q];
    }
    unsigned excl = 0;
    if (tile > 0) {
      unsigned tb = tile - 1;
      while (true) {
        const unsigned v = __hip_atomic_load(status + (uint64_t)tb * 256 + d, __ATOMIC_RELAXED,
                                             __HIP_MEMORY_SCOPE_AGENT);
        const unsigned f = v >> 30;
        if (f == 0) {
          __builtin_amdgcn_s_sleep(1);
          continue;
        }
        excl += v & kOsMask;
        if (f == 2) break;
        --tb;
      }
      __hip_atomic_store(my, kOsPrefix | (excl + tot), __ATOMIC_RELAXED, __HIP_MEMORY_SCOPE_AGENT);
    }
    goff[d] = cbase + excl - dstart;
  }
  __syncthreads();
#pragma unroll
  for (int r = 0; r < kS2Rows; ++r) {
    const uint64_t i = s2_elem(tile, w, r, l);
    if (i < n) {
      const unsigned d = cls_digit(c[r]);
      const unsigned sidx = wcnt[w][d] + local[r];
      stage[sidx] = c[r];
      if (label_of != nullptr) label_of[i] = d != 0 ? (int32_t)(first_label + goff[d] + sidx) : -1;
      if (big_src != nullptr && d == 0) big_src[goff[0] + sidx] = (int32_t)i;
      if (d == 0) out_cnts[goff[0] + sidx] = cnts[i];
    }
  }
  __syncthreads();
  const unsigned tile_n = (unsigned)(n - tile_base < (uint64_t)kS2Tile ? n - tile_base : kS2Tile);
#pragma unroll 4
  for (int j = 0; j < kS2Rows; ++j) {
    const unsigned idx = j * kS2BS + threadIdx.x;
    if (idx < tile_n) {
      const uint64_t v = stage[idx];
      const unsigned d = cls_digit(v);
      if (big_src != nullptr && d != 0) continue;
      const unsigned dst = goff[d] + idx;
      const int32_t key = comp_key(v);
      out_keys[dst] = key;
      if (d != 0) out_cnts[dst] = comp_cnt(v);
      if (key == INT32_MIN && d != 0 && sentinel_label != nullptr) {
        *sentinel_label = first_label + (int64_t)dst;
      } else if (table != nullptr && d != 0) {
        const int64_t label = first_label + (int64_t)dst;
        {
          const unsigned long long want = ((unsigned long long)(uint32_t)label << 32) | (uint32_t)key;
          uint64_t slot = (uint64_t)slot_hash(key) & mask;
          while (atomicCAS(&table[slot], kEncEmptySlot, want) != kEncEmptySlot) slot = (slot + 1) & mask;
        }
      }
    }
  }
}

__global__ __launch_bounds__(kS2BS) void cls_scatter_kernel(
    const int32_t *__restrict__ keys, const int64_t *__restrict__ cnts, uint64_t n,
    const unsigned *__restrict__ cls_hist, unsigned *status, unsigned *ticket, int32_t *out_keys,
    int64_t *out_cnts, unsigned long long *table, uint64_t mask, int64_t first_label,
    int64_t *sentinel_label, int32_t *label_of) {
  cls_scatter_body(keys, cnts, n, cls_hist, status, ticket, out_keys, out_cnts, table, mask,
                   first_label, sentinel_label, label_of);
}

constexpr int kOrdBatch = 16;
struct OrdJob {
  const int32_t *keys;
  const int64_t *cnts;
  const unsigned *cls_hist;
  unsigned *status, *ticket;
  int32_t *out_keys;
  int64_t *out_cnts;
  int32_t *label_of;
  unsigned long long *table;
  int64_t *sentinel_label;
  int32_t *aux;
  unsigned long long *fb_status;
  unsigned long long n, capacity, nslots, flat_slots, first_label, status_words, fb_words;
};
struct OrdBatch {
  OrdJob j[kOrdBatch];
  unsigned tile_start[kOrdBatch + 1];
  unsigned flat_start[kOrdBatch + 1];
  int njobs;
};
__device__ __forceinline__ int ord_job_of(const unsigned *start, int n, unsigned b) {
  int c = 0;
  while (c + 1 < n && b >= start[c + 1]) ++c;
  return c;
}

__global__ __launch_bounds__(kBlock) void ord_prep_kernel(OrdBatch b) {
  const OrdJob &j = b.j[blockIdx.y];
  const uint64_t stride = (uint64_t)gridDim.x * kBlock;
  const uint64_t t0 = (uint64_t)blockIdx.x * kBlock + threadIdx.x;
  for (uint64_t i = t0; i < j.status_words; i += stride) j.status[i] = 0;
  for (uint64_t i = t0; i < j.fb_words; i += stride) j.fb_status[i] = 0;
  if (j.flat_slots) {
    for (uint64_t i = t0; i < j.capacity; i += stride) j.table[i] = kEncEmptySlot;
  }
  if (t0 == 0) *j.sentinel_label = -1;
}

__global__ __launch_bounds__(kS2BS) void cls_scatter_many_kernel(OrdBatch b) {
  const int ji = ord_job_of(b.tile_start, b.njobs, blockIdx.x);
  const OrdJob &j = b.j[ji];
  cls_scatter_body(j.keys, j.cnts, j.n, j.cls_hist, j.status, j.ticket, j.out_keys, j.out_cnts,
                   nullptr, 0, (int64_t)j.first_label, j.sentinel_label, j.label_of);
}

__device__ __forceinline__ void range_patch_body(unsigned long long *table, uint64_t nslots,
                                                 const int32_t *__restrict__ label_of) {
  const uint64_t stride = (uint64_t)gridDim.x * kBlock * 2;
  for (uint64_t s0 = ((uint64_t)blockIdx.x * kBlock + threadIdx.x) * 2; s0 < nslots; s0 += stride) {
    ulonglong2 e = *reinterpret_cast<ulonglong2 *>(table + s0);
    bool dirty = false;
    if ((int32_t)(uint32_t)e.x != INT32_MIN) {
      e.x = ((unsigned long long)(uint32_t)label_of[(uint32_t)(e.x >> 32)] << 32) | (uint32_t)e.x;
      dirty = true;
    }
    if ((int32_t)(uint32_t)e.y != INT32_MIN) {
      e.y = ((unsigned long long)(uint32_t)label_of[(uint32_t)(e.y >> 32)] << 32) | (uint32_t)e.y;
      dirty = true;
    }
    if (dirty) *reinterpret_cast<ulonglong2 *>(table + s0) = e;
  }
}
__global__ __launch_bounds__(kBlock) void range_patch_kernel(unsigned long long *table,
                                                             uint64_t nslots,
                                                             const int32_t *__restrict__ label_of) {
  range_patch_body(table, nslots, label_of);
}

__global__ __launch_bounds__(kBlock) void range_fix_prefix_kernel(
    unsigned long long *table, const int32_t *__restrict__ aux, const int32_t *__restrict__ vocab,
    uint64_t n_big, int64_t first_label, int64_t *sentinel_label, uint64_t table_slots) {
  const RangeMap map = load_map(aux);
  const uint64_t stride = (uint64_t)gridDim.x * kBlock;
  for (uint64_t j = (uint64_t)blockIdx.x * kBlock + threadIdx.x; j < n_big; j += stride) {
    const int32_t key = vocab[j];
    const int64_t label = first_label + (int64_t)j;
    if (key == INT32_MIN) {
      *sentinel_label = label;
      continue;
    }
    uint64_t s = map.table_slot(key);
    if (map.flat) {
      s = flat_find_from(table, table_slots, s, key, table[s]);
      if (s != ~0ull) table[s] = ((unsigned long long)(uint32_t)label << 32) | (uint32_t)key;
      continue;
    }
    while (true) {
      const unsigned long long e = table[s];
      if ((int32_t)(uint32_t)e == key) {
        table[s] = ((unsigned long long)(uint32_t)label << 32) | (uint32_t)key;
        break;
      }
      if ((int32_t)(uint32_t)e == INT32_MIN) break;
      ++s;
    }
  }
}

__global__ __launch_bounds__(kBlock) void range_patch_many_kernel(OrdBatch b) {
  const OrdJob &j = b.j[blockIdx.y];
  if (j.flat_slots || j.nslots == 0) return;
  range_patch_body(j.table, j.nslots, j.label_of);
}

struct FixJob {
  unsigned long long *table;
  const int32_t *aux, *vocab;
  int64_t *sentinel_label;
  unsigned long long n_big, first_label, table_slots;
};
struct FixBatch {
  FixJob j[kOrdBatch];
};
__global__ __launch_bounds__(kBlock) void range_fix_prefix_many_kernel(FixBatch b) {
  const FixJob &f = b.j[blockIdx.y];
  const RangeMap map = load_map(f.aux);
  const uint64_t stride = (uint64_t)gridDim.x * kBlock;
  for (uint64_t j = (uint64_t)blockIdx.x * kBlock + threadIdx.x; j < f.n_big; j += stride) {
    const int32_t key = f.vocab[j];
    const int64_t label = (int64_t)f.first_label + (int64_t)j;
    if (key == INT32_MIN) {
      *f.sentinel_label = label;
      continue;
    }
    uint64_t s = map.table_slot(key);
    if (map.flat) {
      s = flat_find_from(f.table, f.table_slots, s, key, f.table[s]);
      if (s != ~0ull) f.table[s] = ((unsigned long long)(uint32_t)label << 32) | (uint32_t)key;
      continue;
    }
    while (true) {
      const unsigned long long e = f.table[s];
      if ((int32_t)(uint32_t)e == key) {
        f.table[s] = ((unsigned long long)(uint32_t)label << 32) | (uint32_t)key;
        break;
      }
      if ((int32_t)(uint32_t)e == INT32_MIN) break;
      ++s;
    }
  }
}

__global__ __launch_bounds__(kBlock) void class_hist_kernel(const int64_t *__restrict__ cnts,
                                                            uint64_t n, unsigned *hist) {
  __shared__ unsigned h[256];
  h[threadIdx.x] = 0;
  __syncthreads();
  const uint64_t stride = (uint64_t)gridDim.x * kBlock;
  unsigned ones = 0;
  for (uint64_t i = (uint64_t)blockIdx.x * kBlock + threadIdx.x; i < n; i += stride) {
    const int64_t c = cnts[i];
    if (c == 1)
      ++ones;
    else
      atomicAdd(&h[c < 255 ? (c < 0 ? 0 : (unsigned)c) : 255u], 1u);
  }
#pragma unroll
  for (int off = 32; off > 0; off >>= 1) ones += __shfl_down(ones, off, 64);
  if (lane_id() == 0 && ones) atomicAdd(&h[1], ones);
  __syncthreads();
  if (h[threadIdx.x]) atomicAdd(&hist[threadIdx.x], h[threadIdx.x]);
}

__device__ __forceinline__ void flat_params_body(const int32_t *__restrict__ keys, uint64_t n,
                                                 uint64_t slots, int32_t *aux) {
  const uint64_t first = (n > 1 && keys[0] == INT32_MIN) ? 1 : 0;
  const uint64_t lo = ukey(keys[first]), hi = ukey(keys[n - 1]);
  const uint64_t span = hi - lo, F = slots;
  uint32_t mul;
  int sh;
  range_map_params(span, F, &mul, &sh);
  aux[NVT_RANGE_AUX_LO] = (int32_t)(uint32_t)lo;
  aux[NVT_RANGE_AUX_LO + 1] = (int32_t)(uint32_t)span;
  aux[NVT_RANGE_AUX_LO + 2] = (int32_t)mul;
  aux[NVT_RANGE_AUX_LO + 3] = 0;
  aux[NVT_RANGE_AUX_LO + 4] = sh;
  aux[NVT_RANGE_AUX_LO + 5] = 1;
  aux[NVT_RANGE_AUX_LO + 6] = keys[0] == INT32_MIN ? 1 : 0;
  aux[NVT_FLAT_AUX_MAXDISP] = 0;
}
__global__ void flat_params_kernel(const int32_t *__restrict__ keys, uint64_t n, uint64_t slots,
                                   int32_t *aux) {
  flat_params_body(keys, n, slots, aux);
}
// ... 122 lines not shown
  const uint64_t stride = (uint64_t)gridDim.x * kBlock;
  for (uint64_t i = (uint64_t)blockIdx.x * kBlock + threadIdx.x; i < n; i += stride) {
    const int32_t k = keys[i];
    const uint32_t l = (uint32_t)labels[i];
    out_keys[l] = k;
    out_cnts[l] = cnts[i];
    abs_label[i] = (int32_t)(first_label + (int64_t)l);
    if (k == INT32_MIN && sentinel_label != nullptr) *sentinel_label = first_label + (int64_t)l;
  }
}

struct OrderWs {
  unsigned *status, *ticket, *fb_ticket;
  char *sort_tmp;
  int32_t *label_of;
  unsigned long long *fb_status;
  uint64_t ntiles, status_bytes, fb_bytes, bytes;
};
static OrderWs order_ws(void *tmp, uint64_t n, uint64_t n_big) {
  OrderWs w;
  w.ntiles = (n + kS2Tile - 1) / kS2Tile;
  w.status_bytes = w.ntiles * 256 * 4 + 64;
  w.fb_bytes = w.ntiles * 8 + 64;
  uint64_t sort_bytes = 0;
  if (n_big > 1) (void)nvt_vocab_sort_tmp_bytes(4, n_big, &sort_bytes);
  const uint64_t sort_at = pad16(w.status_bytes), label_at = sort_at + pad16(sort_bytes),
                 fb_at = label_at + pad16(n * 4);
  const uintptr_t base = reinterpret_cast<uintptr_t>(tmp);
  w.status = reinterpret_cast<unsigned *>(base);
  w.ticket = w.status + w.ntiles * 256;
  w.sort_tmp = reinterpret_cast<char *>(base + sort_at);
  w.label_of = reinterpret_cast<int32_t *>(base + label_at);
  w.fb_status = reinterpret_cast<unsigned long long *>(base + fb_at);
  w.fb_ticket = reinterpret_cast<unsigned *>(w.fb_status + w.ntiles);
  w.bytes = fb_at + pad16(w.fb_bytes) + 64;
  return w;
}

int vocab_from_labels(const int32_t *src_keys, const int64_t *src_cnts, const int32_t *labels, uint64_t n,
                      int32_t *out_keys, int64_t *out_cnts, void *tmp, int64_t first_label, void *table,
                      uint64_t capacity, int64_t *sentinel_label, const int32_t *range_aux,
                      uint64_t flat_slots, hipStream_t s) {
  if (n == 0) return NVT_OK;
  NVT_CHECK_ARG(n < (1ull << 30), "at most 2^30-1 vocabulary entries");
  const OrderWs w = order_ws(tmp, n, 0);
  int32_t *abs_label = w.label_of;
  const bool flat = table != nullptr && range_aux != nullptr && flat_slots > 0;
  if (table != nullptr) {
    if (flat) {
      NVT_CHECK_ARG(flat_slots >= 64 && flat_slots < (1ull << 32), "flat table: 64 .. 2^32-1 slots");
      NVT_CHECK_ARG(capacity >= flat_slots + n + 64, "flat table: slots + n + 64");
    }
    int rc = encode_clear_any(4, table, capacity, sentinel_label, s);
    if (rc) return rc;
  }
  NVT_PROF("vocab_order", 0, s);
  label_scatter_kernel<<<stream_grid(n, kBlock, 8), kBlock, 0, s>>>(src_keys, src_cnts, labels, n, first_label,
                                                                    out_keys, out_cnts, abs_label,
                                                                    table != nullptr ? sentinel_label : nullptr);
  NVT_CHECK_LAUNCH();
  if (flat) {
    int32_t *aux = const_cast<int32_t *>(range_aux);
    flat_params_kernel<<<1, 1, 0, s>>>(src_keys, n, flat_slots, aux);
    NVT_CHECK_LAUNCH();
    NVT_CHECK_HIP(hipMemsetAsync(w.fb_status, 0, w.fb_bytes, s));
    flat_build_kernel<<<(unsigned)w.ntiles, kS2BS, 0, s>>>(src_keys, abs_label, n, aux, w.fb_status,
                                                          w.fb_ticket, (unsigned long long *)table,
                                                          capacity);
    NVT_CHECK_LAUNCH();
  } else if (table != nullptr) {
    int rc = encode_insert_any(4, out_keys, n, first_label, table, capacity, sentinel_label, s);
    if (rc) return rc;
  }
  return NVT_OK;
}

uint64_t vocab_order_tmp_bytes(uint64_t n, uint64_t n_big) { return order_ws(nullptr, n, n_big).bytes; }

int vocab_order_from_sorted(const int32_t *src_keys, const int64_t *src_cnts, uint64_t n,
                            const unsigned *cls_hist, uint64_t n_big, int64_t max_count,
                            int32_t *out_keys, int64_t *out_cnts, void *tmp, int64_t first_label,
                            void *table, uint64_t capacity, int64_t *sentinel_label,
                            const int32_t *range_aux, int range_nb_log2, hipStream_t s,
                            bool *tail_deferred, uint64_t flat_slots) {
  *tail_deferred = false;
  if (n == 0) return NVT_OK;
  NVT_CHECK_ARG(n < (1ull << 30), "at most 2^30-1 vocabulary entries");
  NVT_CHECK_ARG(n_big <= n, "n_big > n");
  const OrderWs w = order_ws(tmp, n, n_big);
  const bool flat = table != nullptr && range_aux != nullptr && flat_slots > 0;
  const bool ranged = table != nullptr && range_aux != nullptr;
  if (flat) {
    NVT_CHECK_ARG(flat_slots >= 64 && flat_slots < (1ull << 32), "flat table: 64 .. 2^32-1 slots");
    NVT_CHECK_ARG(capacity >= flat_slots + n + 64, "flat table: slots + n + 64");
    int rc = encode_clear_any(4, table, capacity, sentinel_label, s);
    if (rc) return rc;
  } else if (table && !ranged) {
    int rc = encode_clear_any(4, table, capacity, sentinel_label, s);
    if (rc) return rc;
  } else if (ranged) {
    NVT_CHECK_HIP(hipMemsetAsync(sentinel_label, 0xFF, 8, s));
  }
  {
    NVT_PROF("vocab_order", 0, s);
    NVT_CHECK_HIP(hipMemsetAsync(w.status, 0, w.status_bytes, s));
    cls_scatter_kernel<<<(unsigned)w.ntiles, kS2BS, 0, s>>>(
        src_keys, src_cnts, n, cls_hist, w.status, w.ticket, out_keys, out_cnts,
        ranged ? nullptr : (unsigned long long *)table, capacity - 1, first_label, sentinel_label,
        ranged ? w.label_of : nullptr);
    NVT_CHECK_LAUNCH();
    if (flat) {
      int32_t *aux = const_cast<int32_t *>(range_aux);
      flat_params_kernel<<<1, 1, 0, s>>>(src_keys, n, flat_slots, aux);
      NVT_CHECK_LAUNCH();
      NVT_CHECK_HIP(hipMemsetAsync(w.fb_status, 0, w.fb_bytes, s));
      flat_build_kernel<<<(unsigned)w.ntiles, kS2BS, 0, s>>>(
          src_keys, w.label_of, n, aux, w.fb_status, w.fb_ticket, (unsigned long long *)table, capacity);
      NVT_CHECK_LAUNCH();
    } else if (ranged) {
      const uint64_t nslots = ((uint64_t)1 << range_nb_log2) * kRpRegion + kRpGuard;
      range_patch_kernel<<<stream_grid(nslots / 2, kBlock, 8), kBlock, 0, s>>>(
          (unsigned long long *)table, nslots, w.label_of);
      NVT_CHECK_LAUNCH();
    }
  }
  if (vocab_sort_small_eligible(4, n_big, max_count)) {
    *tail_deferred = true;
    return NVT_OK;
  }
  if (n_big > 1) {
    int rc = vocab_sort_any(4, out_keys, out_cnts, n_big, max_count, w.sort_tmp, s);
    if (rc) return rc;
  }
  if (table && n_big > 0) {
    if (ranged) {
      NVT_PROF("encode_build", 0, s);
      range_fix_prefix_kernel<<<stream_grid(n_big, kBlock), kBlock, 0, s>>>(
          (unsigned long long *)table, range_aux, out_keys, n_big, first_label, sentinel_label,
          capacity);
      NVT_CHECK_LAUNCH();
    } else {
      int rc = encode_insert_any(4, out_keys, n_big, first_label, table, capacity, sentinel_label, s);
      if (rc) return rc;
    }
  }
  return NVT_OK;
}

int vocab_order_sorted_batch(const OrderSortedJob *jobs, int njobs, hipStream_t s) {
  for (int j0 = 0; j0 < njobs; j0 += kOrdBatch) {
    const int nj = njobs - j0 < kOrdBatch ? njobs - j0 : kOrdBatch;
    OrdBatch b;
    memset(&b, 0, sizeof(b));
    std::vector<OrderTail> tails;
    OrderWs ws[kOrdBatch];
    bool any_flat = false, any_ranged = false;
    for (int i = 0; i < nj; ++i) {
      const OrderSortedJob &q = jobs[j0 + i];
      NVT_CHECK_ARG(q.n > 0 && q.n < (1ull << 30), "1 .. 2^30-1 vocabulary entries");
      NVT_CHECK_ARG(q.n_big <= q.n, "n_big > n");
      NVT_CHECK_ARG(q.table && q.range_aux && q.tmp && q.sentinel_label, "range table jobs only");
      const OrderWs &w = ws[i] = order_ws(q.tmp, q.n, q.n_big);
      OrdJob &o = b.j[i];
      o.keys = q.src_keys;
      o.cnts = q.src_cnts;
      o.cls_hist = q.cls_hist;
      o.status = w.status;
      o.ticket = w.ticket;
      o.out_keys = q.out_keys;
      o.out_cnts = q.out_cnts;
      o.label_of = w.label_of;
      o.table = reinterpret_cast<unsigned long long *>(q.table);
      o.sentinel_label = q.sentinel_label;
      o.aux = const_cast<int32_t *>(q.range_aux);
      o.fb_status = w.fb_status;
      o.n = q.n;
      o.capacity = q.capacity;
      o.flat_slots = q.flat_slots;
      o.nslots = q.flat_slots ? 0 : ((uint64_t)1 << q.range_nb_log2) * kRpRegion + kRpGuard;
      o.first_label = (unsigned long long)q.first_label;
      o.status_words = w.status_bytes / 4;
      o.fb_words = q.flat_slots ? w.fb_bytes / 8 : 0;
      if (q.flat_slots) {
        NVT_CHECK_ARG(q.flat_slots >= 64 && q.flat_slots < (1ull << 32), "flat table: 64 .. 2^32-1 slots");
        NVT_CHECK_ARG(q.capacity >= q.flat_slots + q.n + 64, "flat table: slots + n + 64");
        any_flat = true;
      } else {
        any_ranged = true;
      }
      b.tile_start[i + 1] = b.tile_start[i] + (unsigned)w.ntiles;
      b.flat_start[i + 1] = b.flat_start[i] + (q.flat_slots ? (unsigned)w.ntiles : 0u);
    }
    b.njobs = nj;
    {
      NVT_PROF("vocab_order", 0, s);
      ord_prep_kernel<<<dim3(any_flat ? 2048 : 64, nj), kBlock, 0, s>>>(b);
      NVT_CHECK_LAUNCH();
      cls_scatter_many_kernel<<<b.tile_start[nj], kS2BS, 0, s>>>(b);
      NVT_CHECK_LAUNCH();
      if (any_flat) {
        flat_params_many_kernel<<<nj, 1, 0, s>>>(b);
        NVT_CHECK_LAUNCH();
        flat_build_many_kernel<<<b.flat_start[nj], kS2BS, 0, s>>>(b);
        NVT_CHECK_LAUNCH();
      }
      if (any_ranged) {
        range_patch_many_kernel<<<dim3(1024, nj), kBlock, 0, s>>>(b);
        NVT_CHECK_LAUNCH();
      }
    }
    for (int i = 0; i < nj; ++i) {
      const OrderSortedJob &q = jobs[j0 + i];
      if (q.n_big == 0) continue;
      if (vocab_sort_small_eligible(4, q.n_big, q.max_count)) {
        tails.push_back({q.out_keys, q.out_cnts, q.n_big, q.first_label, q.table, q.capacity,
                         q.sentinel_label, q.range_aux});
        continue;
      }
      if (q.n_big > 1) {
        int rc = vocab_sort_any(4, q.out_keys, q.out_cnts, q.n_big, q.max_count, ws[i].sort_tmp, s);
        if (rc) return rc;
      }
      NVT_PROF("encode_build", 0, s);
      range_fix_prefix_kernel<<<stream_grid(q.n_big, kBlock), kBlock, 0, s>>>(
          (unsigned long long *)q.table, q.range_aux, q.out_keys, q.n_big, q.first_label,
          q.sentinel_label, q.capacity);
      NVT_CHECK_LAUNCH();
    }
    if (!tails.empty()) {
      int rc = vocab_order_tail_batch(tails.data(), (int)tails.size(), s);
      if (rc) return rc;
    }
  }
  return NVT_OK;
}

int vocab_order_tail_batch(const OrderTail *t, int nt, hipStream_t s) {
  if (nt == 0) return NVT_OK;
  std::vector<SmallSortDesc> d(nt);
  for (int i = 0; i < nt; ++i) {
    d[i].keys = t[i].keys;
    d[i].counts = t[i].counts;
    d[i].n = (unsigned)t[i].n_big;
  }
  int rc = vocab_sort_small_batch(d.data(), nt, s);
  if (rc) return rc;
  NVT_PROF("encode_build", 0, s);
  for (int i0 = 0; i0 < nt;) {
    FixBatch fb;
    memset(&fb, 0, sizeof(fb));
    int nf = 0;
    uint64_t longest = 0;
    for (; i0 < nt && nf < kOrdBatch; ++i0) {
      if (!t[i0].table || !t[i0].range_aux) continue;
      fb.j[nf++] = {(unsigned long long *)t[i0].table, t[i0].range_aux, t[i0].keys,
                    t[i0].sentinel_label, t[i0].n_big, (unsigned long long)t[i0].first_label,
                    t[i0].capacity};
      longest = t[i0].n_big > longest ? t[i0].n_big : longest;
    }
    if (nf) {
      range_fix_prefix_many_kernel<<<dim3(stream_grid(longest, kBlock), nf), kBlock, 0, s>>>(fb);
      NVT_CHECK_LAUNCH();
    }
  }
  for (int i = 0; i < nt; ++i) {
    if (!t[i].table) continue;
    if (t[i].range_aux) {
      continue;
    } else {
      rc = encode_insert_any(4, t[i].keys, t[i].n_big, t[i].first_label, t[i].table, t[i].capacity,
                             t[i].sentinel_label, s);
      if (rc) return rc;
    }
  }
  return NVT_OK;
}

}

using namespace nvt;

extern "C" {

int nvt_class_hist(const int64_t *counts, uint64_t n, uint32_t *hist, void *stream) {
  NVT_CHECK_ARG(hist && (n == 0 || counts), "null pointer");
  hipStream_t s = (hipStream_t)stream;
  NVT_CHECK_HIP(hipMemsetAsync(hist, 0, 256 * 4, s));
  if (n == 0) return NVT_OK;
  class_hist_kernel<<<stream_grid(n, kBlock * 8, 4), kBlock, 0, s>>>(counts, n, hist);
  NVT_CHECK_LAUNCH();
  return NVT_OK;
}
int nvt_vocab_label_shard(const int32_t *keys, const int64_t *counts, uint64_t n, const uint32_t *class_base_diff,
                          void *tmp, int32_t *label_of, int32_t *big_keys, int64_t *big_counts,
                          int32_t *big_src, void *stream) {
  if (n == 0) return NVT_OK;
  NVT_CHECK_ARG(keys && counts && class_base_diff && tmp && label_of && big_keys && big_counts && big_src,
                "null pointer");
  NVT_CHECK_ARG(n < (1ull << 30), "at most 2^30-1 entries");
  hipStream_t s = (hipStream_t)stream;
  const OrderWs w = order_ws(tmp, n, 0);
  NVT_PROF("vocab_order", 0, s);
  NVT_CHECK_HIP(hipMemsetAsync(w.status, 0, w.status_bytes, s));
  label_shard_kernel<<<(unsigned)w.ntiles, kS2BS, 0, s>>>(keys, counts, n, class_base_diff, w.status,
                                                         w.ticket, big_keys, big_counts, label_of, big_src);
  NVT_CHECK_LAUNCH();
  return NVT_OK;
}

int nvt_vocab_order_tmp_bytes(uint64_t n, uint64_t n_big, uint64_t *bytes) {
  NVT_CHECK_ARG(bytes, "null out pointer");
  *bytes = vocab_order_tmp_bytes(n, n_big);
  return NVT_OK;
}

int nvt_flat_index_tmp_bytes(uint64_t n, uint64_t *bytes) {
  NVT_CHECK_ARG(bytes, "null out");
  const uint64_t ntiles = (n + kS2Tile - 1) / kS2Tile;
  *bytes = pad16(ntiles * 8 + 64) + 64;
  return NVT_OK;
}

int nvt_flat_index_build(const int32_t *keys, uint64_t n, uint64_t slots, int32_t *aux, void *table,
                         uint64_t capacity, void *tmp, void *stream) {
  NVT_CHECK_ARG(keys && aux && table && tmp, "null pointer");
  NVT_CHECK_ARG(n >= 1 && n < (1ull << 30), "1 .. 2^30-1 keys");
// ... 20 lines not shown
```

### nvtabular_amd/kernels_count.py

```python
from __future__ import annotations

import ctypes as C
import math
import os
from typing import List, NamedTuple, Optional, Sequence, Tuple

import torch

from . import _lib
from . import kernels as K
from ._lib import check

MIN_COUNT_CAPACITY = 1 << 16


class CountTable:

    def __init__(self, key_dtype: torch.dtype, capacity: int, device=None):
        _lib.require_gpu()
        self.lib = _lib.load()
        self.key_dtype = key_dtype
        self.key_bytes = 4 if key_dtype == torch.int32 else 8
        self.suffix = "i32" if self.key_bytes == 4 else "i64"
        self.capacity = K.next_pow2(capacity)
# ... 161 lines not shown

def _range_bits(s) -> int:
    want = max(1, -(-max(s.hint, 1) // RANGE_KEYS_PER_BUCKET))
    return max(s.min_range_bits, min(10, max(8, (want - 1).bit_length())))


def _launch_path_of(s, path: int) -> int:
    if path == PATH_RANGE:
        return PATH_RANGE | (_range_bits(s) << 8) | (PATH_PIECES if s.pieces is not None else 0)
    eligible = path in (1, 2, 3) and s.kb == 4 and not s.weighted
    return path | PATH_HOT if eligible and (s.hot is None or s.hot) else path


def escalate(s: CountPolicy, ovf: int, need: int):
    if ovf & 1:
        if s.path == PATH_SORT:
            raise _lib.NvtHipError("dense count: the sort path reported a table overflow")
        int32_plain = s.kb == 4 and not s.weighted
        if s.path == PATH_RANGE:
            if _range_bits(s) < 10:
                return s._replace(min_range_bits=10, cap_guess=max(s.cap_guess, 1 << 22))
            if not s.range_failed:
                s = s._replace(range_failed=True, range_fail_bits=int(ovf))
            nxt = 1
        elif s.path == 0 and s.allow_range and int32_plain and not s.range_failed:
            return s._replace(path=PATH_RANGE, cap_guess=max(s.cap_guess, 1 << 20))
        elif s.path == PATH_ORDER[-1]:
            return FALLBACK
        else:
            nxt = PATH_ORDER[PATH_ORDER.index(s.path) + 1]
        if nxt == 7 and _launch_path_of(s, 1) & PATH_HOT:
            nxt = 1
        if nxt == 1 and s.range_failed and int32_plain:
            nxt = PATH_SORT
        elif nxt == 1 and s.hint > PATH_P1_MAX_DISTINCT:
            nxt = 2 if s.hint <= PATH_P2_MAX_DISTINCT else 3
        return s._replace(path=nxt, cap_guess=max(s.cap_guess, _path_max()[nxt]))
    if ovf & 2:
        if s.cap_guess > s.n:
            raise _lib.NvtHipError("dense count: output list overflowed at full capacity")
        exact = need if s.path in (PATH_RANGE, PATH_SORT) else 0
        return s._replace(cap_guess=exact + 64 if exact > s.cap_guess else max(4 * s.cap_guess, 1 << 20))
    return DONE


def assign_streams(paths, ns, streams: int, head_start: bool):
    m = len(paths)
    order = list(range(m))
    if streams == 1 or m < 2:
        return order, [0] * m
    head = 0
    if head_start:
        free = [i for i in order if paths[i] in _S_CLASSES][:streams]
        if free and len(free) < m:
            order = free + [i for i in order if i not in free]
            if len(free) == streams and paths[order[-1]] not in _S_CLASSES:
                head = streams
    cost = [_PATH_COST.get(paths[i], 1.0) * ns[i] for i in order]
    slots, load = list(range(head)) + [0] * (m - head), [0.0] * streams
    for k in range(head):
        load[k] += cost[k]
    for k in sorted(range(head, m), key=lambda k: -cost[k]):
        slots[k] = load.index(min(load))
        load[slots[k]] += cost[k]
    return order, slots


def _plain_info(path: int, distinct: int, max_count: int, rows: int) -> dict:
    return dict(path=path, distinct=distinct, max_count=max_count, rows=rows)


def _empty_result(keys: torch.Tensor):
    return (torch.empty(0, dtype=keys.dtype, device=keys.device),
            torch.empty(0, dtype=torch.int64, device=keys.device), 0, _plain_info(0, 0, 0, 0))


class DenseCountJob:

    def __init__(self, keys, valid, weights=None, hint: int = 0, allow_range: bool = True,
                 pieces=None, min_range_bits: int = 8):
        _lib.require_gpu()
        self.want_table = True
        self.range_table = None
        self.allow_range = allow_range
        self.range_failed = False
        self.range_fail_bits = 0
        self.pieces = pieces
        self.min_range_bits = max(8, min(10, int(min_range_bits)))
        self.lib = _lib.load()
        self.keys = K.aligned(keys)
        self.valid = valid
        self.weights = weights.contiguous() if weights is not None else None
        self.weighted = weights is not None
        self.n = int(self.keys.numel())
        self.dev = self.keys.device
        self.suffix = K._key_suffix(self.keys)
        self.kb = 4 if self.suffix == "i32" else 8
        self.hint = hint
        self.path = _path_for(hint, small_tables=(self.weighted or self.kb == 8),
                              allow_range=allow_range)
        self.cap_guess = max(1 << 16, 2 * max(hint, 1))
        self.state = None
        self.result = None
        self.hot = None

    def range_bits(self) -> int:
        return _range_bits(self)

    def _policy(self) -> CountPolicy:
        return CountPolicy(*[getattr(self, f) for f in CountPolicy._fields])

    def prepare(self, desc: "_lib.CountCol") -> int:
        n, path = self.n, self.path
        out_cap = min(self.cap_guess, n) + 1
        if path in _S_CLASSES:
            out_cap = min(out_cap, _S_CLASSES[path] * 256 * 384 + 1)
        self.out_k = torch.empty(out_cap + 1, dtype=self.keys.dtype, device=self.dev)
        self.out_c = torch.empty(out_cap + 1, dtype=torch.int64, device=self.dev)
        lpath = _launch_path_of(self, path)
        key = (self.kb, n, lpath, self.weighted)
        nbytes = _WS_BYTES.get(key)
        if nbytes is None:
            out = C.c_uint64()
            check(self.lib.nvt_dense_count_ws_bytes(self.kb, n, lpath, int(self.weighted), C.byref(out)))
            nbytes = _WS_BYTES[key] = out.value
        desc.keys = self.keys.data_ptr()
        desc.valid = K.ptr(self.valid)
        desc.weights = K.ptr(self.weights)
        desc.n = n
        desc.key_bytes = self.kb
        desc.path = lpath
        desc.out_keys = self.out_k.data_ptr()
        desc.out_counts = self.out_c.data_ptr()
        desc.out_capacity = out_cap
        desc.state = self.state.data_ptr()
        desc.hot_image = None
        desc.range_table = None
        if path == PATH_SORT:
            self.hot_image = torch.empty(256, dtype=torch.int32, device=self.dev)
            desc.hot_image = self.hot_image.data_ptr()
        elif path == PATH_RANGE:
            self.hot_image = torch.empty(RANGE_AUX_WORDS, dtype=torch.int32, device=self.dev)
            if self.pieces is not None:
                self.hot_image[RANGE_AUX_PW:RANGE_AUX_PW + K.RANGE_PIECES + 1] = self.pieces
            desc.hot_image = self.hot_image.data_ptr()
            if self.want_table:
                bits = self.range_bits()
                rt_bytes = _RT_BYTES.get(bits)
                if rt_bytes is None:
                    rt_out = C.c_uint64()
                    check(self.lib.nvt_range_table_bytes(bits, C.byref(rt_out)))
                    rt_bytes = _RT_BYTES[bits] = rt_out.value
                self.range_table = torch.empty(rt_bytes, dtype=torch.uint8, device=self.dev)
                self.table_bits = bits
                desc.range_table = self.range_table.data_ptr()
        elif lpath & PATH_HOT:
            self.hot_image = torch.empty(HOT_IMAGE_WORDS, dtype=torch.int32, device=self.dev)
            desc.hot_image = self.hot_image.data_ptr()
        return nbytes

    def resolve(self, st) -> bool:
        ovf = st[_lib.ST_OVERFLOW]
        nxt = escalate(self._policy(), ovf, st[_lib.ST_NEED]) if ovf else DONE
        if nxt is FALLBACK:
            self._fallback()
            return True
        if nxt is not DONE:
            self.path, self.cap_guess, self.min_range_bits = nxt.path, nxt.cap_guess, nxt.min_range_bits
            self.range_failed, self.range_fail_bits = nxt.range_failed, nxt.range_fail_bits
            return False
        m = st[_lib.ST_OCCUPIED]
        max_count = st[_lib.ST_MAXCOUNT]
        if self.path not in (PATH_RANGE, PATH_SORT) and st[_lib.ST_SENTINEL] > 0:
            self.out_k[m] = K.INT32_MIN if self.kb == 4 else K.INT64_MIN
            self.out_c[m] = st[_lib.ST_SENTINEL]
            max_count = max(max_count, st[_lib.ST_SENTINEL])
            m += 1
        self.result = (self.out_k[:m], self.out_c[:m], st[_lib.ST_NULLS], self._info(st, m, max_count))
        return True

    def _info(self, st, m: int, max_count: int) -> dict:
        info = _plain_info(self.path, m, max_count, st[_lib.ST_ROWS])
        info["range_fail_bits"] = self.range_fail_bits
        if self.path != PATH_RANGE:
            info["range_failed"] = self.range_failed
        if self.path in (PATH_RANGE, PATH_SORT):
            info.update(sorted_by_key=True, cls_hist=self.hot_image, n_big=st[_lib.ST_BIG],
                        range_pieces=self.pieces is not None)
        if self.path == PATH_RANGE:
            info.update(cls_hist=self.hot_image[RANGE_AUX_HIST:RANGE_AUX_HIST + 256],
                        range_aux=self.hot_image, range_table=self.range_table,
                        range_bits=self.table_bits if self.range_table is not None else 0,
                        range_bits_floor=self.min_range_bits)
        return info

    def _fallback(self):
        if self.weights is None:
            tab, st = count_into_new_table([self.keys], [self.valid], max(self.hint, 1 << 20))
        else:
            keys, weights, null_weight = self.keys, self.weights, 0
            if self.valid is not None:
                ok = K.unpack_bitmap(self.valid, self.n)
                null_weight = int(weights[~ok].sum().item())
                keys, weights = keys[ok].contiguous(), weights[ok].contiguous()
            tab = CountTable(torch.int64, 2 * max(int(keys.numel()), 1))
            if keys.numel():
                tab.merge(keys.to(torch.int64), weights)
            st = tab.read_state()
            st[_lib.ST_NULLS] += null_weight
        k, c = tab.compact()
        k = k.to(self.keys.dtype)
        mx = int(c.max().item()) if c.numel() else 0
        self.result = (k, c, st[_lib.ST_NULLS], _plain_info(-1, int(k.numel()), mx, self.n))


def _estimate_distinct(d: int, m: int, n: int) -> int:
    if m <= 0 or d <= 0:
        return 1
    r = d / m
    if r < 0.02:
        D = float(d)
    elif r > 0.999:
        D = float(n)
    else:
        lo, hi = 1e-6, 60.0
        for _ in range(60):
            mid = 0.5 * (lo + hi)
            if (1.0 - math.exp(-mid)) / mid > r:
                lo = mid
            else:
                hi = mid
        D = m / (0.5 * (lo + hi))
    return int(min(n, 3.0 * D + 64))


def _presample(jobs):
    cand = [j for j in jobs if j.result is None and j.hint <= 0 and j.weights is None
            and j.n >= SAMPLE_MIN_ROWS]
    if not cand:
        return
    if K.PRESAMPLE_SKETCH:
        descs = (_lib.PrefixCol * len(cand))()
        for d, j in zip(descs, cand):
            d.keys, d.valid = j.keys.data_ptr(), K.ptr(j.valid)
            d.n, d.key_bytes = min(SAMPLE_ROWS, j.n), j.kb
        out = torch.empty((len(cand), 2), dtype=torch.int64, device=cand[0].dev)
        check(cand[0].lib.nvt_prefix_distinct(descs, len(cand), out.data_ptr(), K.stream_ptr()),
              "nvt_prefix_distinct")
        res = [(None, None, 0, dict(distinct=int(d), rows=int(r))) for d, r in K.read_back(out).tolist()]
    else:
        samples = []
        for j in cand:
            valid = None if j.valid is None else j.valid[: SAMPLE_ROWS // 8]
            sj = DenseCountJob(j.keys[:SAMPLE_ROWS], valid, None, hint=SAMPLE_ROWS)
            sj.path, sj.cap_guess = 1, SAMPLE_ROWS
            samples.append(sj)
        res = CountBatch(samples, presample=False).results()
    for j, (_, _, nulls, info) in zip(cand, res):
        est = _estimate_distinct(info["distinct"], info["rows"] - nulls, j.n)
        j.hint = est
        K.stat_add("presampled_columns")
        seen_rows = max(int(info["rows"]) - int(nulls), 1)
        j.min_range_bits = max(j.min_range_bits, 10 if int(info["distinct"]) * 10 >= seen_rows else 8)
        j.path = _path_for(est, small_tables=(j.kb == 8), allow_range=j.allow_range)
        j.cap_guess = max(1 << 16, 2 * est, j.n // 6 if j.path not in _S_CLASSES else 0)


class CountBatch:

    def __init__(self, jobs, presample: bool = True):
        self.jobs = list(jobs)
        self._results = None
        if presample:
            _presample(self.jobs)
# ... 139 lines not shown
```

### nvtabular_amd/kernels_encode.py

```python
from __future__ import annotations

import ctypes as C
from typing import List, Optional

import torch

from . import _lib
from . import kernels as K
from ._lib import check

ENCODE_RESIDENT_I32, ENCODE_RESIDENT_I64 = 8192, 6144
_BYTES = {}


def encode_kind(key_bytes: int, n_vocab: int, unique: bool, defer_build: bool, has_range_table: bool,
                flat: bool) -> str:
    resident = K.ENCODE_RESIDENT_I32 if key_bytes == 4 else K.ENCODE_RESIDENT_I64
    if unique and 0 < n_vocab <= resident:
        return "resident"
    if has_range_table:
        assert defer_build and unique and key_bytes == 4
        return "dumped"
    if flat and defer_build and unique and key_bytes == 4:
        return "flat"
    if unique and n_vocab > 0:
        return "cache" if key_bytes == 4 else "linear64"
    return "generic"


def encode_launch_shape(kind: str, key_bytes: int, out_bytes: int, n_vocab: int, has_head_image: bool) -> str:
    if kind == "generic":
        return "encode_kernel"
    if kind == "resident":
        if key_bytes == 4 and out_bytes == 8 and n_vocab <= 2048:
            return "encode_small_kernel<2048>" if n_vocab <= 1024 else "encode_small_kernel<4096>"
        return "encode_hot_kernel<GLOBAL=false>"
    if kind == "linear64":
        return "encode_hot_kernel<int64,GLOBAL=true>"
    if kind in ("flat", "dumped"):
        return "encode_pipe_kernel<2>" if kind == "flat" else "encode_pipe_kernel<1>"
    return "cache mode, head image" if has_head_image else "cache mode, head per launch"


def _lib_bytes(name: str, *args) -> int:
    key = (name,) + args
    if key not in _BYTES:
        out = C.c_uint64()
        check(getattr(_lib.load(), name)(*args, C.byref(out)), name)
        _BYTES[key] = out.value
    return _BYTES[key]


class EncodeTable:

    FLAT_AUX_WORDS, FLAT_AUX_MAXDISP = 8192 + 16, 8192 + 8
    FLAT_MAX_DISPLACEMENT = 4096

    def __init__(self, vocab_keys: torch.Tensor, first_label: int, unique: bool = False,
                 defer_build: bool = False, range_table=None, flat: bool = False):
        _lib.require_gpu()
        self.suffix = K._key_suffix(vocab_keys)
        self.key_dtype = vocab_keys.dtype
        self.key_bytes = 4 if self.suffix == "i32" else 8
        self.n_vocab = n = int(vocab_keys.numel())
        self.first_label = int(first_label)
        self.unique = bool(unique)
        self.kind = kind = encode_kind(self.key_bytes, n, self.unique, bool(defer_build),
                                       range_table is not None, bool(flat))
        dev = vocab_keys.device
        self._vk = vk = vocab_keys.contiguous()
        self.vocab_keys = vk if unique else None
        self.sort_tmp = None
        self._counts = None
        self._src = None
        self.ready = None
        self.pending = False
        self._release = False
        self.table = self.range_aux = None
        self.range_bits = self.flat_slots = 0
        self.capacity = K.next_pow2(max(64, (4 if n <= (1 << 20) else 2) * n + 1))
        hashed = kind in ("generic", "cache", "linear64")
        if kind == "dumped":
            self.table, self.range_aux, self.range_bits = range_table
            self.capacity = 0
        elif kind == "flat":
            self.flat_slots = max(64, int(n / K.FLAT_INDEX_LOAD) + 1)
            self.capacity = self.flat_slots + n + 64
            self.table = torch.empty(self.capacity * 8, dtype=torch.uint8, device=dev)
            self.range_aux = torch.empty(self.FLAT_AUX_WORDS, dtype=torch.int32, device=dev)
        elif hashed:
            nbytes = _lib_bytes("nvt_encode_table_bytes", self.key_bytes, self.capacity)
            self.table = torch.empty(nbytes, dtype=torch.uint8, device=dev)
        self.sentinel_label = None if kind == "resident" else torch.empty(1, dtype=torch.int64, device=dev)
        self.head_image = None
        if defer_build and kind in ("cache", "flat", "dumped"):
            self.head_image = torch.empty(_lib.ENCODE_HEAD_BYTES, dtype=torch.uint8, device=dev)
        if hashed and not defer_build:
            check(
                getattr(_lib.load(), f"nvt_encode_build_{self.suffix}")(
                    vk.data_ptr() if n else None, n, self.first_label, self.table.data_ptr(),
                    self.capacity, self.sentinel_label.data_ptr(), 1 if unique else 0, K.stream_ptr(),
                ),
                "nvt_encode_build",
            )

    def fill_vocab_desc(self, d: "_lib.VocabCol", counts: torch.Tensor, max_count: int, src=None):
        n = self.n_vocab
        src_keys = src_counts = cls_hist = labels = None
        n_big = 0
        if src is not None:
            src_keys, src_counts, cls_hist, n_big = src[:4]
            labels = src[4] if len(src) > 4 else None
            if labels is not None:
                assert labels.dtype == torch.int32 and labels.numel() == src_keys.numel()
                labels, n_big = labels.contiguous(), 0
                K.stat_add("labelled_vocabularies")
            assert self.key_bytes == 4 and self.unique and src_keys.numel() == n and counts.numel() == n
            self._src = (src_keys, src_counts, cls_hist, labels)
            scratch = _lib_bytes("nvt_vocab_order_tmp_bytes", n, int(n_big))
        else:
            small = self.key_bytes == 4 and 2 <= n <= 16384 and 0 < int(max_count) < (1 << 32)
            scratch = _lib_bytes("nvt_vocab_sort_tmp_bytes", self.key_bytes, n) if n > 1 and not small else None
        self._counts = counts
        d.keys = self._vk.data_ptr()
        d.counts = counts.data_ptr()
        d.n = n
        d.max_count = int(max_count)
        d.key_bytes = self.key_bytes
        d.unique_keys = 1 if self.unique else 0
        d.src_keys, d.src_counts = K.ptr(src_keys), K.ptr(src_counts)
        d.cls_hist, d.src_labels = K.ptr(cls_hist), K.ptr(labels)
        d.n_big = int(n_big)
        d.range_aux = K.ptr(self.range_aux)
        d.range_nb_log2 = int(self.range_bits)
        d.flat_slots = int(self.flat_slots)
        if scratch is not None:
            self.sort_tmp = torch.empty(scratch + 16, dtype=torch.uint8, device=self._vk.device)
        d.sort_tmp = K.ptr(self.sort_tmp) if scratch is not None else None
        d.first_label = self.first_label
        d.table = K.ptr(self.table)
        d.capacity = self.capacity
        d.sentinel_label = K.ptr(self.sentinel_label)
        d.head_image = K.ptr(self.head_image)
        if scratch is not None and K.ASYNC_FINALIZE:
            if self.ready is None:
                self.ready = K.Event()
            d.ready_event = self.ready.handle
            self.pending = True
        else:
            d.ready_event = None

    def flat_ok(self) -> bool:
        self.wait_ready()
        return int(self.range_aux[self.FLAT_AUX_MAXDISP].item()) & 0xFFFFFFFF <= self.FLAT_MAX_DISPLACEMENT

    def _drop_ordering(self):
        self.sort_tmp = None
        self._counts = None
        self._src = None

    def wait_ready(self):
        if self.pending:
            self.ready.wait()
            self.pending = False
            self._drop_ordering()

    def __del__(self):
        try:
            if getattr(self, "pending", False):
                self.wait_ready()
        except Exception:
            pass

    def fill_encode_desc(self, d: "_lib.EncodeCol", keys, valid, null_label, oov_label,
                         num_buckets, out):
        d.keys = keys.data_ptr()
        d.valid = K.ptr(valid)
        d.n = keys.numel()
        d.table = K.ptr(self.table)
        d.capacity = self.capacity
        d.sentinel_label = K.ptr(self.sentinel_label)
        d.null_label = int(null_label)
        d.oov_label = int(oov_label)
        d.num_buckets = int(num_buckets or 0)
        d.key_bytes = self.key_bytes
        d.out_bytes = out.element_size()
        d.out = out.data_ptr()
        d.vocab_keys = K.ptr(self.vocab_keys) if self.n_vocab else None
        d.n_vocab = self.n_vocab if self.vocab_keys is not None else 0
        d.first_label = self.first_label
        d.range_aux = K.ptr(self.range_aux)
        d.head_image = K.ptr(self.head_image)
        if self.pending:
            d.wait_event = self.ready.handle
            self.pending = False
            self._release = True
        else:
            d.wait_event = None

    def release_ordering(self):
        if self._release:
            self._release = False
            self._drop_ordering()

    def encode(self, keys: torch.Tensor, valid: Optional[torch.Tensor], null_label: int, oov_label: int,
               num_buckets: int = 0, out_dtype: torch.dtype = torch.int64) -> torch.Tensor:
        return encode_many([(self, keys, valid, null_label, oov_label, num_buckets)], out_dtype)[0]


def flat_tables_ok(tabs) -> List[bool]:
    dev = tabs[0].range_aux.device
    side = K._check_streams.get(dev.index)
    if side is None:
        side = K._check_streams[dev.index] = torch.cuda.Stream(device=dev)
    for t in tabs:
        if t.ready is not None:
            t.ready.wait(stream=side.cuda_stream)
        else:
            side.wait_stream(torch.cuda.current_stream(dev))
    with torch.cuda.stream(side):
        words = torch.stack([t.range_aux[EncodeTable.FLAT_AUX_MAXDISP] for t in tabs]).to(torch.int64)
        vals = K.read_back(words)
    return [(int(d) & 0xFFFFFFFF) <= EncodeTable.FLAT_MAX_DISPLACEMENT for d in vals]


def encode_many(items, out_dtype: torch.dtype = torch.int64):
    if out_dtype not in (torch.int32, torch.int64):
        raise TypeError("Categorify output dtype must be int32 or int64")
    order = sorted(range(len(items)),
                   key=lambda i: (1, -items[i][0].n_vocab) if items[i][0].pending else (0, 0))
    descs = (_lib.EncodeCol * max(1, len(items)))()
    outs, keep = [None] * len(items), []
    for d, i in zip(descs, order):
        tab, keys, valid, null_label, oov_label, nb = items[i]
        if keys.dtype != tab.key_dtype:
            keys = keys.to(tab.key_dtype)
        keys = K.aligned(keys)
        out = torch.empty(keys.numel(), dtype=out_dtype, device=keys.device)
        tab.fill_encode_desc(d, keys, valid, null_label, oov_label, nb, out)
        outs[i] = out
        keep.append(keys)
    try:
# ... 31 lines not shown
```

### nvtabular_amd/ops/categorify.py

```python
from __future__ import annotations

import os
import warnings
from copy import deepcopy
from typing import Dict, List

import numpy as np
import pandas as pd
import torch

from .. import kernels as K
from ..device import DeviceColumn, DeviceFrame, as_device_frame, key_view
from ..schema import Tags
from ..selector import ColumnSelector
from .base import StatOperator

PAD_OFFSET = 0
NULL_OFFSET = 1
OOV_OFFSET = 2


def _make_name(*args, sep="_"):
    return sep.join(args)

# ... 335 lines not shown
                bounds.append(int(g.valid_rows))
            if tabs:
                for g, (k, c, sc, info) in zip(singles, dist.merge_counts_many(tabs, key_sorted, bounds)):
                    g.table = (k, c, sc[2])
                    g.nulls, g.valid_rows = sc[0], sc[1]
                    g.any_rank_strings = sc[3] > 0
                    g.merged = True
                    g.sorted = (k, info) if info is not None and info.get("sorted_by_key") else None
        self._complete_sorted_info(groups)
        opts = {}
        for g in groups:
            nb = _pick(self.num_buckets, g.name) if self.num_buckets else None
            oov_count = nb or 1
            max_emb = _pick(self.max_size, g.name) if self.max_size else 0
            freq = _pick(self.freq_threshold, g.name, 0) if self.freq_threshold else 0
            if max_emb and max_emb < oov_count + 2:
                raise ValueError(
                    "`max_size` can never be less than the maximum of `num_buckets + 2` and `3`, "
                    "because we must always reserve pad, null and at least 1 oov-bucket index."
                )
            opts[g.name] = (oov_count, max_emb, freq)
        fast = [g for g in groups if self._fast_finalizable(g, opts[g.name], dist)]
        if fast:
            for g in fast:
                paths[g.name] = "/".join([str(base), f"unique.{g.name}.parquet"])
            if self.defer_artifacts and LAZY_FINALIZE:
                self._lazy_finalize = (fast, opts, base)
            else:
                with K.annotate("write_uniques"):
                    self._finalize_fast(fast, opts, base)
        for g in groups:
            if g.name in paths:
                continue
            oov_count, max_emb, freq = opts[g.name]
            with K.annotate("write_uniques"):
                if g.combo:
                    vocab = self._finalize_combo(g, dist)
                else:
                    vocab = self._finalize_single(g, dist)
                paths[g.name] = self._save_encodings(
                    g, vocab, base, first_n=max_emb, freq_threshold=freq, oov_count=oov_count
                )
        if not self.defer_artifacts:
            dist.barrier()
        return {name: paths[name] for name in state if name in paths}

    def _fast_finalizable(self, g, opt, dist):
        _, max_emb, freq = opt
        if g.combo or g.table is None or max_emb or freq or self.tie_break == "reference":
            return False
        if any(c in g.strings for c in g.cols) or getattr(g, "any_rank_strings", False):
            return False
        if dist.world_size() > 1 and not getattr(g, "merged", False):
            return False
        return int(g.table[0].numel()) > 0

    def _ensure_finalized(self, small_only=False):
        if self._lazy_finalize is None:
            return
        groups, opts, base = self._lazy_finalize
        if small_only:
            now = [g for g in groups if _small_vocab(g)]
            rest = [g for g in groups if not _small_vocab(g)]
            self._lazy_finalize = (rest, opts, base) if rest else None
        else:
            now, self._lazy_finalize = groups, None
        if now:
            with K.annotate("write_uniques"):
                self._finalize_fast(now, opts, base)

    def _finalize_fast(self, groups, opts, base):
        descs = (K._lib.VocabCol * len(groups))()
        built = []
        for d, g in zip(descs, groups):
            keys, counts, max_count = g.table
            keys, counts = keys.contiguous(), counts.contiguous()
            start = opts[g.name][0] + OOV_OFFSET
            src = rtab = None
            if g.sorted is not None and g.sorted[0] is g.table[0] and keys.dtype == torch.int32:
                info = g.sorted[1]
                src = (keys, counts, info["cls_hist"], info["n_big"], info.get("label_of"))
                keys, counts = torch.empty_like(keys), torch.empty_like(counts)
                if info.get("range_table") is not None:
                    rtab = (info["range_table"], info["range_aux"], info["range_bits"])
            tab = K.EncodeTable(keys, start, unique=True, defer_build=True, range_table=rtab,
                                flat=src is not None and rtab is None and g.name not in self._no_flat)
            tab.fill_vocab_desc(d, counts, max_count, src=src)
            built.append((g, keys, counts, tab, start))
        K.check(K._lib.load().nvt_vocab_finalize_many(descs, len(groups), K.stream_ptr()),
                "nvt_vocab_finalize_many")
        self._flat_unchecked = [g.name for g, _, _, tab, _ in built if tab.flat_slots]
        for g, keys, counts, tab, start in built:
            if not tab.pending:
                tab._drop_ordering()
            self._encoders[g.name] = _SingleEncoder(tab, start)
            n = int(counts.numel())
            final = dict(
                name=g.name, cols=list(g.cols), combo=False, keys=[keys], null_mask=None,
                counts=counts, strings=None, start=start, oov_count=opts[g.name][0], oov_size=0,
                unique_count=n, unique_size=int(g.valid_rows), null_size=g.nulls,
                empty_input=False, base=str(base), table=tab,
            )
            if self.defer_artifacts:
                self._pending[g.name] = final
            elif self._is_writer:
                _write_artifacts(final)
            else:
                tab.wait_ready()

    def _check_flat_tables(self):
        names, self._flat_unchecked = self._flat_unchecked, []
        todo = [(n, self._encoders[n]) for n in names
                if n in self._encoders and getattr(self._encoders[n].table, "flat_slots", 0)]
        if not todo:
            return
        for (name, enc), ok in zip(todo, K.flat_tables_ok([e.table for _, e in todo])):
            if ok:
                continue
            self._no_flat.add(name)
            final = self._pending.get(name)
            keys = final["keys"][0] if final is not None else enc.table._vk
            tab = K.EncodeTable(keys, enc.first_label_in_file, unique=True)
            self._encoders[name] = _SingleEncoder(tab, enc.first_label_in_file)
            if final is not None:
                final["table"] = tab

    def _finalize_single(self, g: _GroupFit, dist):
        if g.table is None:
            dev = torch.device("cuda", torch.cuda.current_device())
            keys = torch.empty(0, dtype=torch.int64, device=dev)
            counts = torch.empty(0, dtype=torch.int64, device=dev)
            max_count = 0
        else:
            keys, counts, max_count = g.table
        nulls = g.nulls
        if dist.world_size() > 1 and not getattr(g, "merged", False):
            keys, counts, nulls = dist.merge_counts(keys, counts, nulls)
            tot = dist.all_reduce_sum(torch.tensor([max_count, g.valid_rows], dtype=torch.int64,
                                                   device=keys.device)).tolist()
            max_count, g.valid_rows = int(tot[0]), int(tot[1])
        strings = None
        for c in g.cols:
            if c in g.strings:
                strings = {**(strings or {}), **g.strings[c]}
        strings = dist.merge_string_luts(strings)
        if self.tie_break == "reference" and keys.numel():
            hk, hc = K.read_back(keys.to(torch.int64)), K.read_back(counts)
            vals = np.array([strings[int(k)] for k in hk], dtype=object) if strings is not None else hk
            df = pd.DataFrame({"v": vals, "k": hk, "s": hc})
            df = df.sort_values(["v"], na_position="first", ignore_index=True)
            df = df.sort_values("s", ascending=False, ignore_index=True)
            keys = torch.from_numpy(df["k"].to_numpy().astype(hk.dtype)).to(keys.device).to(keys.dtype)
            counts = torch.from_numpy(df["s"].to_numpy().astype(np.int64)).to(counts.device)
        elif strings is not None:
            hk, hc = keys.cpu().numpy(), counts.cpu().numpy()
            vals = np.array([strings[int(k)] for k in hk], dtype=object)
            order = np.lexsort((vals, -hc))
            keys = torch.from_numpy(hk[order]).to(keys.device)
            counts = torch.from_numpy(hc[order]).to(counts.device)
        else:
            keys, counts = keys.contiguous(), counts.contiguous()
            K.vocab_sort(keys, counts, max_count)
        return dict(keys=[keys], null_mask=None, counts=counts, null_size=nulls, strings=strings,
                    total=g.valid_rows)

    def _finalize_combo(self, g: _GroupFit, dist):
        if g.table is None:
# ... 533 lines not shown
```

Before: 4.970 billion rows/s.

## Record range-table slots at count time and chunk small vocab sorts

The range count kernel now records each unique key's slot in the range table, so vocab ordering can write labels straight into that slot. This removes the separate range_patch pass for those columns. Separately, the small-vocabulary sort splits columns larger than 2048 entries into 2048-entry bitonic chunks spread over many blocks, then merges them with a binary-search rank kernel, instead of sorting each column in a single block. The change adds a scratch buffer, an extra slot array, and an extra kernel launch.

```diff
diff --git a/include/nvt_hip.h b/include/nvt_hip.h
--- a/include/nvt_hip.h
+++ b/include/nvt_hip.h
@@ -384,6 +384,7 @@
   uint64_t *state;
   int32_t *hot_image;
   void *range_table;
+  uint32_t *out_slots;
 } nvt_count_col;
 int nvt_range_table_bytes(int nb_log2, uint64_t *bytes);
 int nvt_dense_count_many(const nvt_count_col *cols, int ncols, void *stream);
@@ -409,6 +410,7 @@
   uint64_t flat_slots;
   const int32_t *src_labels;
   void *head_image;
+  const uint32_t *src_slots;
 } nvt_vocab_col;
 #define NVT_ENCODE_HEAD_BYTES (12288 * 12 + 64)
 #define NVT_FLAT_AUX_WORDS (NVT_RANGE_AUX_LO + 16)
diff --git a/nvtabular_amd/_lib.py b/nvtabular_amd/_lib.py
--- a/nvtabular_amd/_lib.py
+++ b/nvtabular_amd/_lib.py
@@ -161,7 +161,7 @@
     _fields_ = [("keys", _vp), ("valid", _vp), ("weights", _vp), ("n", _u64),
                 ("key_bytes", C.c_int32), ("path", C.c_int32), ("ws", _vp), ("out_keys", _vp),
                 ("out_counts", _vp), ("out_capacity", _u64), ("state", _vp), ("hot_image", _vp),
-                ("range_table", _vp)]
+                ("range_table", _vp), ("out_slots", _vp)]
 
 
 class VocabCol(C.Structure):
@@ -171,7 +171,7 @@
                 ("sentinel_label", _vp), ("ready_event", _vp), ("src_keys", _vp),
                 ("src_counts", _vp), ("cls_hist", _vp), ("n_big", _u64), ("range_aux", _vp),
                 ("range_nb_log2", C.c_int32), ("flat_slots", C.c_uint64), ("src_labels", _vp),
-                ("head_image", _vp)]
+                ("head_image", _vp), ("src_slots", _vp)]
 
 
 class MergeCol(C.Structure):
diff --git a/nvtabular_amd/csrc/nvt_dense_count.hip b/nvtabular_amd/csrc/nvt_dense_count.hip
--- a/nvtabular_amd/csrc/nvt_dense_count.hip
+++ b/nvtabular_amd/csrc/nvt_dense_count.hip
@@ -82,7 +82,7 @@
                             (int32_t *)c.out_keys, c.out_counts, c.out_capacity, c.state, s);
     return range_count_i32((const int32_t *)c.keys, c.valid, c.n, p.nb_log2, c.ws, c.hot_image,
                            (int32_t *)c.out_keys, c.out_counts, c.out_capacity, c.range_table,
-                           c.state, s, p.pieces);
+                           c.out_slots, c.state, s, p.pieces);
   }
   NVT_PROF(prof_name(p), c.n * c.key_bytes, s);
   if (clear_state) NVT_CHECK_HIP(hipMemsetAsync(c.state, 0, NVT_STATE_WORDS * 8, s));
diff --git a/nvtabular_amd/csrc/nvt_finalize.hip b/nvtabular_amd/csrc/nvt_finalize.hip
--- a/nvtabular_amd/csrc/nvt_finalize.hip
+++ b/nvtabular_amd/csrc/nvt_finalize.hip
@@ -97,6 +97,7 @@
       d[j].keys = (int32_t *)c.keys;
       d[j].counts = c.counts;
       d[j].n = (unsigned)c.n;
+      d[j].tmp = c.sort_tmp;
     }
     int rc = vocab_sort_small_batch(d.data(), (int)d.size(), main_s);
     if (rc) return rc;
@@ -119,7 +120,7 @@
       NVT_CHECK_ARG(c.sort_tmp, "null sort_tmp");
       jobs.push_back({(const int32_t *)c.src_keys, c.src_counts, c.n, c.cls_hist, c.n_big, c.max_count,
                       (int32_t *)c.keys, c.counts, c.sort_tmp, c.first_label, c.table, c.capacity,
-                      c.sentinel_label, c.range_aux, c.range_nb_log2, c.flat_slots});
+                      c.sentinel_label, c.range_aux, c.range_nb_log2, c.flat_slots, c.src_slots});
       job_cols.push_back(i);
       batched[i] = 1;
     }
@@ -162,11 +163,11 @@
                                        c.n_big, c.max_count, (int32_t *)c.keys, c.counts,
                                        c.sort_tmp, c.first_label, c.table, c.capacity,
                                        c.sentinel_label, c.range_aux, c.range_nb_log2, s,
-                                       &deferred, c.flat_slots);
+                                       &deferred, c.flat_slots, c.src_slots);
       if (rc) return rc;
       if (deferred) {
         tails.push_back({(int32_t *)c.keys, c.counts, c.n_big, c.first_label, c.table, c.capacity,
-                         c.sentinel_label, c.range_aux});
+                         c.sentinel_label, c.range_aux, c.sort_tmp, c.n});
         tail_cols.push_back(big[j]);
         continue;
       }
diff --git a/nvtabular_amd/csrc/nvt_internal.hpp b/nvtabular_amd/csrc/nvt_internal.hpp
--- a/nvtabular_amd/csrc/nvt_internal.hpp
+++ b/nvtabular_amd/csrc/nvt_internal.hpp
@@ -20,6 +20,7 @@
   int32_t *keys;
   int64_t *counts;
   unsigned n;
+  void *tmp;
 };
 bool vocab_sort_small_eligible(int key_bytes, uint64_t n, int64_t max_count);
 int vocab_sort_small_batch(const SmallSortDesc *cols, int ncols, hipStream_t s);
@@ -55,7 +56,7 @@
 uint64_t range_count_ws_bytes(uint64_t n, int nb_log2);
 int range_count_i32(const int32_t *keys, const uint8_t *valid, uint64_t n, int nb_log2, void *ws,
                     int32_t *aux, int32_t *out_keys, int64_t *out_cnt, uint64_t out_cap,
-                    void *range_table, uint64_t *state, hipStream_t s, bool pieces);
+                    void *range_table, uint32_t *out_slots, uint64_t *state, hipStream_t s, bool pieces);
 
 uint64_t sort_count_ws_bytes(uint64_t n);
 int sort_count_i32(const int32_t *keys, const uint8_t *valid, uint64_t n, void *ws, unsigned *hist,
@@ -68,7 +69,8 @@
                             int32_t *out_keys, int64_t *out_cnts, void *tmp, int64_t first_label,
                             void *table, uint64_t capacity, int64_t *sentinel_label,
                             const int32_t *range_aux, int range_nb_log2, hipStream_t s,
-                            bool *tail_deferred, uint64_t flat_slots = 0);
+                            bool *tail_deferred, uint64_t flat_slots = 0,
+                            const uint32_t *src_slots = nullptr);
 struct OrderSortedJob {
   const int32_t *src_keys;
   const int64_t *src_cnts;
@@ -86,6 +88,7 @@
   const int32_t *range_aux;
   int range_nb_log2;
   uint64_t flat_slots;
+  const uint32_t *src_slots;
 };
 int vocab_order_sorted_batch(const OrderSortedJob *jobs, int njobs, hipStream_t s);
 int encode_head_build(const int32_t *vocab_keys, uint64_t n, int64_t first_label, void *image,
@@ -105,6 +108,8 @@
   uint64_t capacity;
   int64_t *sentinel_label;
   const int32_t *range_aux;
+  void *tmp;
+  uint64_t n;
 };
 int vocab_order_tail_batch(const OrderTail *t, int nt, hipStream_t s);
 
diff --git a/nvtabular_amd/csrc/nvt_range_count.hip b/nvtabular_amd/csrc/nvt_range_count.hip
--- a/nvtabular_amd/csrc/nvt_range_count.hip
+++ b/nvtabular_amd/csrc/nvt_range_count.hip
@@ -327,7 +327,7 @@
     const int32_t *__restrict__ aux, const unsigned *__restrict__ hot_tot, int nb_log2,
     unsigned long long *status, unsigned *ticket, int32_t *__restrict__ out_keys,
     int64_t *__restrict__ out_cnt, uint64_t out_cap, unsigned *cls_hist,
-    unsigned long long *__restrict__ range_table, uint64_t *state) {
+    unsigned long long *__restrict__ range_table, uint32_t *__restrict__ out_slots, uint64_t *state) {
   constexpr int NSL = kRpSlots + kRpTail;
   constexpr int NW = kRpBS / kWave;
   __shared__ int32_t lkeys[NSL];
@@ -598,6 +598,7 @@
   if (extra && threadIdx.x == 0) {
     out_keys[base] = kEmpty;
     out_cnt[base] = (int64_t)sent_rows;
+    if (out_slots != nullptr) out_slots[base] = 0xFFFFFFFFu;
     const unsigned cls = sent_rows < 255 ? (unsigned)sent_rows : 255u;
     atomicAdd(&hist[cls], 1u);
     unsigned long long *gm = reinterpret_cast<unsigned long long *>(&state[NVT_ST_MAXCOUNT]);
@@ -681,6 +682,7 @@
       const unsigned c = lcnt[i];
       out_keys[pos] = k;
       out_cnt[pos] = (int64_t)c;
+      if (out_slots != nullptr) out_slots[pos] = b * (unsigned)NSL + (unsigned)i;
       atomicAdd(&hist[c < 255u ? c : 255u], 1u);
       mx = c > mx ? c : mx;
       dump = ((unsigned long long)(uint32_t)pos << 32) | (uint32_t)k;
@@ -749,7 +751,8 @@
 
 int range_count_i32(const int32_t *keys, const uint8_t *valid, uint64_t n, int nb_log2, void *wsp,
                     int32_t *aux, int32_t *out_keys, int64_t *out_cnt, uint64_t out_cap,
-                    void *range_table, uint64_t *state, hipStream_t s, bool pieces) {
+                    void *range_table, uint32_t *out_slots, uint64_t *state, hipStream_t s, bool pieces) {
+  if (range_table == nullptr) out_slots = nullptr;
   NVT_CHECK_ARG(nb_log2 >= 6 && nb_log2 <= kRpMaxNbLog2, "range path: 64 .. 1024 buckets");
   NVT_CHECK_ARG(aux != nullptr, "range path: the column needs its aux block (hot_image)");
   NVT_PROF("dense_count_r9", n * 4, s);
@@ -779,12 +782,12 @@
     rp_count_kernel<true><<<NB, kRpBS, 0, s>>>(w.regions, w.fills, cap, aux, w.hot_tot, nb_log2, w.status,
                                                w.ticket, out_keys, out_cnt, out_cap,
                                                (unsigned *)(aux + NVT_RANGE_AUX_HIST),
-                                               (unsigned long long *)range_table, state);
+                                               (unsigned long long *)range_table, out_slots, state);
   else
     rp_count_kernel<false><<<NB, kRpBS, 0, s>>>(w.regions, w.fills, cap, aux, w.hot_tot, nb_log2, w.status,
                                                 w.ticket, out_keys, out_cnt, out_cap,
                                                 (unsigned *)(aux + NVT_RANGE_AUX_HIST),
-                                                (unsigned long long *)range_table, state);
+                                                (unsigned long long *)range_table, out_slots, state);
   NVT_CHECK_LAUNCH();
   return NVT_OK;
 }
diff --git a/nvtabular_amd/csrc/nvt_sort.hip b/nvtabular_amd/csrc/nvt_sort.hip
--- a/nvtabular_amd/csrc/nvt_sort.hip
+++ b/nvtabular_amd/csrc/nvt_sort.hip
@@ -693,15 +693,26 @@
 }
 
 constexpr int kSmallPackedMax = 16384;
+constexpr int kSmallChunk = 2048, kSmallRankBS = 256;
+constexpr int kSmallMaxChunks = kSmallPackedMax / kSmallChunk;
 struct SmallCol {
   int32_t *keys;
   int64_t *counts;
+  uint64_t *tmp;
   unsigned n;
 };
 constexpr int kSmallBatch = 64;
 struct SmallBatch {
   SmallCol c[kSmallBatch];
+  unsigned chunk_start[kSmallBatch + 1];
+  unsigned rank_start[kSmallBatch + 1];
+  int ncols;
 };
+__device__ __forceinline__ int small_col_of(const unsigned *start, int n, unsigned b) {
+  int c = 0;
+  while (c + 1 < n && b >= start[c + 1]) ++c;
+  return c;
+}
 __global__ __launch_bounds__(kSmallBS) void sort_small_packed_many_kernel(SmallBatch b) {
   __shared__ uint64_t sv[kSmallPackedMax];
   const SmallCol col = b.c[blockIdx.x];
@@ -731,6 +742,95 @@
     col.keys[i] = comp_key(v);
     col.counts[i] = comp_cnt(v);
   }
+}
+
+__global__ __launch_bounds__(kSmallBS) void sort_small_chunk_kernel(SmallBatch b) {
+  __shared__ uint64_t sv[kSmallChunk];
+  const int ci = small_col_of(b.chunk_start, b.ncols, blockIdx.x);
+  const SmallCol col = b.c[ci];
+  const unsigned first = (blockIdx.x - b.chunk_start[ci]) * kSmallChunk;
+  const unsigned n = col.n - first < (unsigned)kSmallChunk ? col.n - first : (unsigned)kSmallChunk;
+  unsigned m = 2;
+  while (m < n) m <<= 1;
+  for (unsigned i = threadIdx.x; i < m; i += kSmallBS)
+    sv[i] = i < n ? comp_make(col.keys[first + i], col.counts[first + i]) : ~0ull;
+  __syncthreads();
+  for (unsigned size = 2; size <= m; size <<= 1) {
+    for (unsigned stride = size >> 1; stride > 0; stride >>= 1) {
+      const bool wide = stride > (unsigned)kWave;
+      if (wide) __syncthreads();
+      for (unsigned t = threadIdx.x; t < m / 2; t += kSmallBS) {
+        const unsigned lo = 2 * t - (t & (stride - 1));
+        const unsigned hi = lo + stride;
+        const bool up = (lo & size) == 0;
+        const uint64_t a = sv[lo], c = sv[hi];
+        if (up ? (c < a) : (a < c)) {
+          sv[lo] = c;
+          sv[hi] = a;
+        }
+      }
+      if (wide) {
+        __syncthreads();
+      } else {
+        __builtin_amdgcn_fence(__ATOMIC_RELEASE, "wavefront");
+        __builtin_amdgcn_wave_barrier();
+        __builtin_amdgcn_fence(__ATOMIC_ACQUIRE, "wavefront");
+      }
+    }
+  }
+  __syncthreads();
+  if (col.n > (unsigned)kSmallChunk) {
+    for (unsigned i = threadIdx.x; i < n; i += kSmallBS) col.tmp[first + i] = sv[i];
+    return;
+  }
+  for (unsigned i = threadIdx.x; i < n; i += kSmallBS) {
+    const uint64_t v = sv[i];
+    col.keys[i] = comp_key(v);
+    col.counts[i] = comp_cnt(v);
+  }
+}
+
+__global__ __launch_bounds__(kSmallRankBS) void sort_small_rank_kernel(SmallBatch b) {
+  const int ci = small_col_of(b.rank_start, b.ncols, blockIdx.x);
+  const SmallCol col = b.c[ci];
+  const unsigned e = (blockIdx.x - b.rank_start[ci]) * kSmallRankBS + threadIdx.x;
+  if (e >= col.n) return;
+  const uint64_t *__restrict__ src = col.tmp;
+  const uint64_t v = src[e];
+  const unsigned own = e / kSmallChunk;
+  const unsigned nchunks = (col.n + kSmallChunk - 1) / kSmallChunk;
+  unsigned lo[kSmallMaxChunks], hi[kSmallMaxChunks];
+#pragma unroll
+  for (int q = 0; q < kSmallMaxChunks; ++q) {
+    const unsigned at = (unsigned)q * kSmallChunk;
+    lo[q] = 0;
+    hi[q] = 0;
+    if ((unsigned)q < nchunks && (unsigned)q != own)
+      hi[q] = col.n - at < (unsigned)kSmallChunk ? col.n - at : (unsigned)kSmallChunk;
+  }
+  for (int step = 0; step < 12; ++step) {
+    unsigned mid[kSmallMaxChunks];
+    uint64_t a[kSmallMaxChunks];
+#pragma unroll
+    for (int q = 0; q < kSmallMaxChunks; ++q) {
+      mid[q] = (lo[q] + hi[q]) >> 1;
+      a[q] = src[lo[q] < hi[q] ? (unsigned)q * kSmallChunk + mid[q] : e];
+    }
+#pragma unroll
+    for (int q = 0; q < kSmallMaxChunks; ++q) {
+      if (lo[q] < hi[q]) {
+        if (a[q] < v || (a[q] == v && (unsigned)q < own))
+          lo[q] = mid[q] + 1;
+        else
+          hi[q] = mid[q];
+      }
+    }
+  }
+  unsigned rank = e - own * kSmallChunk;
+#pragma unroll
+  for (int q = 0; q < kSmallMaxChunks; ++q) rank += lo[q];
+  col.keys[rank] = comp_key(v);
+  col.counts[rank] = comp_cnt(v);
 }
 
 inline uint64_t sort2_tmp_bytes(uint64_t n) {
@@ -884,16 +984,36 @@
 int vocab_sort_small_batch(const SmallSortDesc *cols, int ncols, hipStream_t s) {
   for (int c0 = 0; c0 < ncols; c0 += kSmallBatch) {
     const int nc = ncols - c0 < kSmallBatch ? ncols - c0 : kSmallBatch;
-    SmallBatch b;
+    SmallBatch b, whole;
     memset(&b, 0, sizeof(b));
+    memset(&whole, 0, sizeof(whole));
+    int nb = 0, nw = 0;
     for (int i = 0; i < nc; ++i) {
-      b.c[i].keys = cols[c0 + i].keys;
-      b.c[i].counts = cols[c0 + i].counts;
-      b.c[i].n = cols[c0 + i].n;
-    }
+      const SmallSortDesc &d = cols[c0 + i];
+      if (d.n > (unsigned)kSmallChunk && d.tmp == nullptr) {
+        whole.c[nw++] = {d.keys, d.counts, nullptr, d.n};
+        continue;
+      }
+      b.c[nb] = {d.keys, d.counts, reinterpret_cast<uint64_t *>(d.tmp), d.n};
+      const unsigned chunks = (d.n + kSmallChunk - 1) / kSmallChunk;
+      b.chunk_start[nb + 1] = b.chunk_start[nb] + chunks;
+      b.rank_start[nb + 1] = b.rank_start[nb] + (chunks > 1 ? (d.n + kSmallRankBS - 1) / kSmallRankBS : 0u);
+      ++nb;
+    }
+    b.ncols = nb;
     NVT_PROF("vocab_sort_small", 0, s);
-    sort_small_packed_many_kernel<<<nc, kSmallBS, 0, s>>>(b);
-    NVT_CHECK_LAUNCH();
+    if (b.chunk_start[nb]) {
+      sort_small_chunk_kernel<<<b.chunk_start[nb], kSmallBS, 0, s>>>(b);
+      NVT_CHECK_LAUNCH();
+    }
+    if (b.rank_start[nb]) {
+      sort_small_rank_kernel<<<b.rank_start[nb], kSmallRankBS, 0, s>>>(b);
+      NVT_CHECK_LAUNCH();
+    }
+    if (nw) {
+      sort_small_packed_many_kernel<<<nw, kSmallBS, 0, s>>>(whole);
+      NVT_CHECK_LAUNCH();
+    }
   }
   return NVT_OK;
 }
diff --git a/nvtabular_amd/csrc/nvt_vocab_order.hip b/nvtabular_amd/csrc/nvt_vocab_order.hip
--- a/nvtabular_amd/csrc/nvt_vocab_order.hip
+++ b/nvtabular_amd/csrc/nvt_vocab_order.hip
@@ -17,7 +17,9 @@
     const int32_t *__restrict__ keys, const int64_t *__restrict__ cnts, uint64_t n,
     const unsigned *__restrict__ cls_hist, unsigned *status, unsigned *ticket, int32_t *out_keys,
     int64_t *out_cnts, unsigned long long *table, uint64_t mask, int64_t first_label,
-    int64_t *sentinel_label, int32_t *label_of, int32_t *big_src = nullptr) {
+    int64_t *sentinel_label, int32_t *label_of, int32_t *big_src = nullptr,
+    const uint32_t *__restrict__ src_slots = nullptr, unsigned long long *slot_table = nullptr,
+    uint64_t nslots = 0) {
   constexpr int NW = kS2BS / kWave;
   __shared__ unsigned wcnt[NW][256];
   __shared__ unsigned goff[256];
@@ -124,7 +126,13 @@
       const unsigned d = cls_digit(c[r]);
       const unsigned sidx = wcnt[w][d] + local[r];
       stage[sidx] = c[r];
-      if (label_of != nullptr) label_of[i] = d != 0 ? (int32_t)(first_label + goff[d] + sidx) : -1;
+      const int32_t lab = d != 0 ? (int32_t)(first_label + goff[d] + sidx) : -1;
+      if (src_slots != nullptr) {
+        const uint32_t sl = src_slots[i];
+        if (sl < nslots) reinterpret_cast<uint32_t *>(slot_table + sl)[1] = (uint32_t)lab;
+      } else if (label_of != nullptr) {
+        label_of[i] = lab;
+      }
       if (big_src != nullptr && d == 0) big_src[goff[0] + sidx] = (int32_t)i;
       if (d == 0) out_cnts[goff[0] + sidx] = cnts[i];
     }
@@ -160,9 +168,10 @@
     const int32_t *__restrict__ keys, const int64_t *__restrict__ cnts, uint64_t n,
     const unsigned *__restrict__ cls_hist, unsigned *status, unsigned *ticket, int32_t *out_keys,
     int64_t *out_cnts, unsigned long long *table, uint64_t mask, int64_t first_label,
-    int64_t *sentinel_label, int32_t *label_of) {
+    int64_t *sentinel_label, int32_t *label_of, const uint32_t *__restrict__ src_slots,
+    unsigned long long *slot_table, uint64_t nslots) {
   cls_scatter_body(keys, cnts, n, cls_hist, status, ticket, out_keys, out_cnts, table, mask,
-                   first_label, sentinel_label, label_of);
+                   first_label, sentinel_label, label_of, nullptr, src_slots, slot_table, nslots);
 }
 
 constexpr int kOrdBatch = 16;
@@ -174,6 +183,7 @@
   int32_t *out_keys;
   int64_t *out_cnts;
   int32_t *label_of;
+  const uint32_t *src_slots;
   unsigned long long *table;
   int64_t *sentinel_label;
   int32_t *aux;
@@ -208,7 +218,8 @@
   const int ji = ord_job_of(b.tile_start, b.njobs, blockIdx.x);
   const OrdJob &j = b.j[ji];
   cls_scatter_body(j.keys, j.cnts, j.n, j.cls_hist, j.status, j.ticket, j.out_keys, j.out_cnts,
-                   nullptr, 0, (int64_t)j.first_label, j.sentinel_label, j.label_of);
+                   nullptr, 0, (int64_t)j.first_label, j.sentinel_label, j.label_of, nullptr,
+                   j.src_slots, j.table, j.nslots);
 }
 
 __device__ __forceinline__ void range_patch_body(unsigned long long *table, uint64_t nslots,
@@ -266,7 +277,7 @@
 
 __global__ __launch_bounds__(kBlock) void range_patch_many_kernel(OrdBatch b) {
   const OrdJob &j = b.j[blockIdx.y];
-  if (j.flat_slots || j.nslots == 0) return;
+  if (j.flat_slots || j.nslots == 0 || j.src_slots != nullptr) return;
   range_patch_body(j.table, j.nslots, j.label_of);
 }
 
@@ -555,7 +566,7 @@
                             int32_t *out_keys, int64_t *out_cnts, void *tmp, int64_t first_label,
                             void *table, uint64_t capacity, int64_t *sentinel_label,
                             const int32_t *range_aux, int range_nb_log2, hipStream_t s,
-                            bool *tail_deferred, uint64_t flat_slots) {
+                            bool *tail_deferred, uint64_t flat_slots, const uint32_t *src_slots) {
   *tail_deferred = false;
   if (n == 0) return NVT_OK;
   NVT_CHECK_ARG(n < (1ull << 30), "at most 2^30-1 vocabulary entries");
@@ -563,6 +574,8 @@
   const OrderWs w = order_ws(tmp, n, n_big);
   const bool flat = table != nullptr && range_aux != nullptr && flat_slots > 0;
   const bool ranged = table != nullptr && range_aux != nullptr;
+  const bool slotted = ranged && !flat && src_slots != nullptr;
+  const uint64_t nslots = ((uint64_t)1 << range_nb_log2) * kRpRegion + kRpGuard;
   if (flat) {
     NVT_CHECK_ARG(flat_slots >= 64 && flat_slots < (1ull << 32), "flat table: 64 .. 2^32-1 slots");
     NVT_CHECK_ARG(capacity >= flat_slots + n + 64, "flat table: slots + n + 64");
@@ -580,7 +593,8 @@
     cls_scatter_kernel<<<(unsigned)w.ntiles, kS2BS, 0, s>>>(
         src_keys, src_cnts, n, cls_hist, w.status, w.ticket, out_keys, out_cnts,
         ranged ? nullptr : (unsigned long long *)table, capacity - 1, first_label, sentinel_label,
-        ranged ? w.label_of : nullptr);
+        ranged ? w.label_of : nullptr, slotted ? src_slots : nullptr,
+        slotted ? (unsigned long long *)table : nullptr, slotted ? nslots : 0);
     NVT_CHECK_LAUNCH();
     if (flat) {
       int32_t *aux = const_cast<int32_t *>(range_aux);
@@ -590,8 +604,7 @@
       flat_build_kernel<<<(unsigned)w.ntiles, kS2BS, 0, s>>>(
           src_keys, w.label_of, n, aux, w.fb_status, w.fb_ticket, (unsigned long long *)table, capacity);
       NVT_CHECK_LAUNCH();
-    } else if (ranged) {
-      const uint64_t nslots = ((uint64_t)1 << range_nb_log2) * kRpRegion + kRpGuard;
+    } else if (ranged && !slotted) {
       range_patch_kernel<<<stream_grid(nslots / 2, kBlock, 8), kBlock, 0, s>>>(
           (unsigned long long *)table, nslots, w.label_of);
       NVT_CHECK_LAUNCH();
@@ -627,7 +640,7 @@
     memset(&b, 0, sizeof(b));
     std::vector<OrderTail> tails;
     OrderWs ws[kOrdBatch];
-    bool any_flat = false, any_ranged = false;
+    bool any_flat = false, any_patch = false;
     for (int i = 0; i < nj; ++i) {
       const OrderSortedJob &q = jobs[j0 + i];
       NVT_CHECK_ARG(q.n > 0 && q.n < (1ull << 30), "1 .. 2^30-1 vocabulary entries");
@@ -643,6 +656,7 @@
       o.out_keys = q.out_keys;
       o.out_cnts = q.out_cnts;
       o.label_of = w.label_of;
+      o.src_slots = q.flat_slots ? nullptr : q.src_slots;
       o.table = reinterpret_cast<unsigned long long *>(q.table);
       o.sentinel_label = q.sentinel_label;
       o.aux = const_cast<int32_t *>(q.range_aux);
@@ -658,8 +672,8 @@
         NVT_CHECK_ARG(q.flat_slots >= 64 && q.flat_slots < (1ull << 32), "flat table: 64 .. 2^32-1 slots");
         NVT_CHECK_ARG(q.capacity >= q.flat_slots + q.n + 64, "flat table: slots + n + 64");
         any_flat = true;
-      } else {
-        any_ranged = true;
+      } else if (q.src_slots == nullptr) {
+        any_patch = true;
       }
       b.tile_start[i + 1] = b.tile_start[i] + (unsigned)w.ntiles;
       b.flat_start[i + 1] = b.flat_start[i] + (q.flat_slots ? (unsigned)w.ntiles : 0u);
@@ -677,7 +691,7 @@
         flat_build_many_kernel<<<b.flat_start[nj], kS2BS, 0, s>>>(b);
         NVT_CHECK_LAUNCH();
       }
-      if (any_ranged) {
+      if (any_patch) {
         range_patch_many_kernel<<<dim3(1024, nj), kBlock, 0, s>>>(b);
         NVT_CHECK_LAUNCH();
       }
@@ -687,7 +701,7 @@
       if (q.n_big == 0) continue;
       if (vocab_sort_small_eligible(4, q.n_big, q.max_count)) {
         tails.push_back({q.out_keys, q.out_cnts, q.n_big, q.first_label, q.table, q.capacity,
-                         q.sentinel_label, q.range_aux});
+                         q.sentinel_label, q.range_aux, q.tmp, q.n});
         continue;
       }
       if (q.n_big > 1) {
@@ -715,6 +729,7 @@
     d[i].keys = t[i].keys;
     d[i].counts = t[i].counts;
     d[i].n = (unsigned)t[i].n_big;
+    d[i].tmp = t[i].tmp ? order_ws(t[i].tmp, t[i].n, t[i].n_big).sort_tmp : nullptr;
   }
   int rc = vocab_sort_small_batch(d.data(), nt, s);
   if (rc) return rc;
diff --git a/nvtabular_amd/kernels_count.py b/nvtabular_amd/kernels_count.py
--- a/nvtabular_amd/kernels_count.py
+++ b/nvtabular_amd/kernels_count.py
@@ -267,6 +267,7 @@
         _lib.require_gpu()
         self.want_table = True
         self.range_table = None
+        self.range_slots = None
         self.allow_range = allow_range
         self.range_failed = False
         self.range_fail_bits = 0
@@ -320,7 +321,8 @@
         desc.out_capacity = out_cap
         desc.state = self.state.data_ptr()
         desc.hot_image = None
-        desc.range_table = None
+        desc.range_table = desc.out_slots = None
+        self.range_slots = None
         if path == PATH_SORT:
             self.hot_image = torch.empty(256, dtype=torch.int32, device=self.dev)
             desc.hot_image = self.hot_image.data_ptr()
@@ -339,6 +341,8 @@
                 self.range_table = torch.empty(rt_bytes, dtype=torch.uint8, device=self.dev)
                 self.table_bits = bits
                 desc.range_table = self.range_table.data_ptr()
+                self.range_slots = torch.empty(out_cap + 1, dtype=torch.int32, device=self.dev)
+                desc.out_slots = self.range_slots.data_ptr()
         elif lpath & PATH_HOT:
             self.hot_image = torch.empty(HOT_IMAGE_WORDS, dtype=torch.int32, device=self.dev)
             desc.hot_image = self.hot_image.data_ptr()
@@ -375,6 +379,7 @@
         if self.path == PATH_RANGE:
             info.update(cls_hist=self.hot_image[RANGE_AUX_HIST:RANGE_AUX_HIST + 256],
                         range_aux=self.hot_image, range_table=self.range_table,
+                        range_slots=self.range_slots[:m] if self.range_slots is not None else None,
                         range_bits=self.table_bits if self.range_table is not None else 0,
                         range_bits_floor=self.min_range_bits)
         return info
diff --git a/nvtabular_amd/kernels_encode.py b/nvtabular_amd/kernels_encode.py
--- a/nvtabular_amd/kernels_encode.py
+++ b/nvtabular_amd/kernels_encode.py
@@ -49,6 +49,9 @@
         check(getattr(_lib.load(), name)(*args, C.byref(out)), name)
         _BYTES[key] = out.value
     return _BYTES[key]
+
+
+SMALL_SORT_CHUNK = 2048
 
 
 class EncodeTable:
@@ -76,12 +79,13 @@
         self.ready = None
         self.pending = False
         self._release = False
-        self.table = self.range_aux = None
+        self.table = self.range_aux = self.range_slots = None
         self.range_bits = self.flat_slots = 0
         self.capacity = K.next_pow2(max(64, (4 if n <= (1 << 20) else 2) * n + 1))
         hashed = kind in ("generic", "cache", "linear64")
         if kind == "dumped":
-            self.table, self.range_aux, self.range_bits = range_table
+            self.table, self.range_aux, self.range_bits = range_table[:3]
+            self.range_slots = range_table[3] if len(range_table) > 3 else None
             self.capacity = 0
         elif kind == "flat":
             self.flat_slots = max(64, int(n / K.FLAT_INDEX_LOAD) + 1)
@@ -107,7 +111,7 @@
     def fill_vocab_desc(self, d: "_lib.VocabCol", counts: torch.Tensor, max_count: int, src=None):
         n = self.n_vocab
         src_keys = src_counts = cls_hist = labels = None
-        n_big = 0
+        n_big = small_scratch = 0
         if src is not None:
             src_keys, src_counts, cls_hist, n_big = src[:4]
             labels = src[4] if len(src) > 4 else None
@@ -121,6 +125,8 @@
         else:
             small = self.key_bytes == 4 and 2 <= n <= 16384 and 0 < int(max_count) < (1 << 32)
             scratch = _lib_bytes("nvt_vocab_sort_tmp_bytes", self.key_bytes, n) if n > 1 and not small else None
+            if small and n > SMALL_SORT_CHUNK:
+                small_scratch = 8 * n
         self._counts = counts
         d.keys = self._vk.data_ptr()
         d.counts = counts.data_ptr()
@@ -130,13 +136,19 @@
         d.unique_keys = 1 if self.unique else 0
         d.src_keys, d.src_counts = K.ptr(src_keys), K.ptr(src_counts)
         d.cls_hist, d.src_labels = K.ptr(cls_hist), K.ptr(labels)
+        d.src_slots = None
+        if self.range_slots is not None and src is not None and labels is None:
+            assert self.range_slots.dtype == torch.int32 and self.range_slots.numel() == n
+            d.src_slots = self.range_slots.data_ptr()
         d.n_big = int(n_big)
         d.range_aux = K.ptr(self.range_aux)
         d.range_nb_log2 = int(self.range_bits)
         d.flat_slots = int(self.flat_slots)
         if scratch is not None:
             self.sort_tmp = torch.empty(scratch + 16, dtype=torch.uint8, device=self._vk.device)
-        d.sort_tmp = K.ptr(self.sort_tmp) if scratch is not None else None
+        elif small_scratch:
+            self.sort_tmp = torch.empty(small_scratch + 16, dtype=torch.uint8, device=self._vk.device)
+        d.sort_tmp = K.ptr(self.sort_tmp) if scratch is not None or small_scratch else None
         d.first_label = self.first_label
         d.table = K.ptr(self.table)
         d.capacity = self.capacity
@@ -158,6 +170,7 @@
         self.sort_tmp = None
         self._counts = None
         self._src = None
+        self.range_slots = None
 
     def wait_ready(self):
         if self.pending:
diff --git a/nvtabular_amd/ops/categorify.py b/nvtabular_amd/ops/categorify.py
--- a/nvtabular_amd/ops/categorify.py
+++ b/nvtabular_amd/ops/categorify.py
@@ -441,7 +441,8 @@
                 src = (keys, counts, info["cls_hist"], info["n_big"], info.get("label_of"))
                 keys, counts = torch.empty_like(keys), torch.empty_like(counts)
                 if info.get("range_table") is not None:
-                    rtab = (info["range_table"], info["range_aux"], info["range_bits"])
+                    rtab = (info["range_table"], info["range_aux"], info["range_bits"],
+                            info.get("range_slots"))
             tab = K.EncodeTable(keys, start, unique=True, defer_build=True, range_table=rtab,
                                 flat=src is not None and rtab is None and g.name not in self._no_flat)
             tab.fill_vocab_desc(d, counts, max_count, src=src)
```

Result: faster. 5.061 billion rows/s, median of 6 (+1.8%).
